# FauxFaux/quadrs

Measured on AMD Instinct MI355X. Metric: Msamples/s through shift->FIR->FFT chain, higher is better.
Workload: dtype f32

## Files before the change

quadrs_amd/build.py:

```python
import os
import subprocess
import sys

HERE = os.path.dirname(os.path.abspath(__file__))
ROOT = os.path.dirname(HERE)
SRC = [(os.path.join(HERE, "csrc", "quadrs_hip.hip"), [])]
DEPS = [s for s, _ in SRC] + [os.path.join(HERE, "csrc", f) for f in ("qd_chain.h", "qd_cascade.h", "qd_device.h", "qd_geometry.h", "qd_registry.h", "qd_summary.h", "qd_pieces.h", "qd_pool.h", "qd_limbs.h", "qd_mean.h", "qd_power.h", "qd_spread.h", "qd_density.h", "qd_bands.h", "qd_paint.h", "qd_lists.h", "qd_bursts.h", "qd_emissions.h", "qd_cuts.h", "qd_cuts_plan.h", "qd_symbols.h", "qd_symbols_plan.h")] + [
    os.path.join(ROOT, "include", "quadrs_hip.h")]
OBJ_DIR = os.path.join(ROOT, "build", "obj")
OUT = os.path.join(HERE, "libquadrs_hip.so")

FLAGS = ["-O3", "--offload-arch=gfx950", "-ffp-contract=off", "-fPIC", "-std=c++17",
         "-fno-fast-math", "-Wall", "-Wno-unused-function", "-I", os.path.join(ROOT, "include"),
         "-Rpass-analysis=kernel-resource-usage",
         "-mllvm", "-amdgpu-atomic-optimizer-strategy=None"]
RESOURCES = os.path.join(ROOT, "build", "kernel_resources.json")


def parse_resource_remarks(text):
    import re
    out, cur = {}, None
    for line in text.splitlines():
        m = re.search(r"remark: Function Name: (\S+)", line)
        if m:
            cur = out.setdefault(m.group(1), {})
            continue
        m = re.search(r"remark:\s+(TotalSGPRs|VGPRs|ScratchSize \[bytes/lane\]|Occupancy \[waves/SIMD\]|SGPRs Spill|VGPRs Spill): (\d+)", line)
        if m and cur is not None:
            cur[m.group(1).split(" [")[0]] = int(m.group(2))
    return out


def hipcc():
    for c in (os.environ.get("HIPCC"), "/opt/rocm/bin/hipcc", "hipcc"):
        if c and (os.path.isabs(c) and os.path.exists(c) or not os.path.isabs(c)):
            return c
    return "hipcc"


def needs_build():
# ... 94 lines not shown
```

quadrs_amd/csrc/qd_cascade.h:

```cpp
#pragma once

#include "qd_chain.h"

namespace qd {

constexpr uint32_t kCascadeRow = 512;
constexpr uint32_t kCascadeThreads = 256;
constexpr uint32_t kCascS0 = 1, kCascS1 = 2, kCascL2 = 4, kCascS2 = 8;

struct CascadeParams {
    ChainParams c;
    const float *h1, *h2;
    const double2 *jtab;
    const RowBase *rows[3];
    uint64_t row0[3];
    double ratio0, ratio1, ratio2;
    uint64_t S;
    uint32_t D1, T1, D2, T2;
    uint32_t n2;
    uint32_t M;
    uint32_t inter_elems, src_elems;
    uint32_t dmagic1, dmagic2;
    uint32_t phi2;
    uint32_t flags;
};

__device__ __forceinline__ uint32_t casc_pad(uint32_t m, uint32_t dmagic, uint32_t phi = 0) { return dmagic ? m + __umulhi(m + phi, dmagic) : m; }

__device__ __forceinline__ int casc_fir_class(uint32_t D) { return (D & 1) ? 0 : (D == 2 ? 2 : (D == 4 ? 4 : (D % 8 == 0 ? 8 : -1))); }

template <int DC>
__device__ __forceinline__ float2 casc_fir_full(const float2 *x, const_f32_p h, uint32_t T, uint32_t D) {
    v2f acc = {0.f, 0.f};
    uint32_t j = 0;
    for (; j + 8 <= T; j += 8) {
        const float2 *xp = x + (DC == 0 ? j : j + j / D);
        float2 xv[8];
        float hv[8];
#pragma unroll
        for (uint32_t u = 0; u < 8; ++u) { xv[u] = xp[(DC == 2 || DC == 4) ? u + u / DC : u]; hv[u] = h[j + u]; }
#pragma unroll
        for (uint32_t u = 0; u < 8; ++u) {
            const v2f xx = {xv[u].x, xv[u].y}, hh = {hv[u], hv[u]};
            acc = acc + xx * hh;
        }
    }
// ... 9 lines not shown
    float ar = 0.f, ai = 0.f;
    for (uint32_t j = 0; j < jmax; ++j) {
        const float2 x = base[casc_pad(q0 + j, dmagic, phi)];
        const float hj = h[j];
        ar = ar + x.x * hj;
        ai = ai + x.y * hj;
    }
    return make_float2(ar, ai);
}

__device__ __forceinline__ float2 casc_fir(int cls, const float2 *base, uint32_t q0, uint32_t jmax, uint32_t T, uint32_t D, const_f32_p h,
                                           uint32_t dmagic, uint32_t phi) {
    if (jmax == T) {
        const float2 *x = base + casc_pad(q0, dmagic, phi);
        switch (cls) {
        case 0: return casc_fir_full<0>(x, h, T, D);
        case 2: return casc_fir_full<2>(x, h, T, D);
        case 4: return casc_fir_full<4>(x, h, T, D);
        case 8: return casc_fir_full<8>(x, h, T, D);
        default: break;
        }
    }
    return casc_fir_any(base, q0, jmax, h, dmagic, phi);
}

template <int FMT>
__device__ __forceinline__ float2 casc_load(const uint8_t *src, uint64_t i) {
    if constexpr (FMT == 0) return reinterpret_cast<const float2 *>(src)[i];
    else if constexpr (FMT == 1) { const uint16_t w = reinterpret_cast<const uint16_t *>(src)[i]; return make_float2(unpack_cs8(w & 0xff), unpack_cs8(w >> 8)); }
    else if constexpr (FMT == 2) { const uint16_t w = reinterpret_cast<const uint16_t *>(src)[i]; return make_float2(unpack_cu8(w & 0xff), unpack_cu8(w >> 8)); }
    else { const uint32_t w = reinterpret_cast<const uint32_t *>(src)[i]; return make_float2(unpack_cs16(w & 0xffffu), unpack_cs16(w >> 16)); }
}

__device__ __forceinline__ float2 casc_nco(const RowBase *rb, uint64_t row0, uint64_t n, const double2 *jt, double ratio) {
    const uint32_t j = (uint32_t)(n % kCascadeRow);
    const double2 cs = jt[j];
    LaneRot lr;
    lr.jf = (double)j; lr.c = cs.x; lr.s = cs.y;
    return nco_mul<true>(rb[n / kCascadeRow - row0], lr, ratio);
}

template <int FMT>
__global__ __launch_bounds__(kCascadeThreads) void k_cascade(const CascadeParams P) {
    extern __shared__ __attribute__((aligned(16))) float2 casc_lds[];
    float2 *inter = casc_lds;
    float2 *tile = casc_lds + P.inter_elems;
    const uint32_t tid = threadIdx.x;
    const ChainParams &C = P.c;
    const DynGeo geo(C);
    const uint32_t D1 = P.D1, T1 = P.T1, D2 = P.D2, T2 = P.T2, n2 = P.n2, W = C.W;
    const uint32_t c1 = T1 - T1 / 2, c2 = T2 - T2 / 2;
    const uint64_t n1 = (uint64_t)n2 * D1 + T1;
    const bool l2 = (P.flags & kCascL2) != 0;
    const_f32_p h1 = (const_f32_p)P.h1;
    const_f32_p h2 = (const_f32_p)P.h2;
    const uint32_t log_width = 2 * geo.layers;
    const int cls1 = casc_fir_class(D1), cls2 = casc_fir_class(D2);
    for (uint64_t w = C.first_window + blockIdx.x; w < C.first_window + C.n_windows; w += gridDim.x) {
        const uint64_t o = w * P.S;
        const uint64_t b2 = l2 ? o * D2 : o;
        const uint64_t b1 = b2 * D1;
        for (uint32_t i0 = 0; i0 < n2; i0 += P.M) {
            const uint32_t m = n2 - i0 < P.M ? n2 - i0 : P.M;
            const uint64_t s0 = b1 + (uint64_t)i0 * D1 + c1;
            const uint64_t want = (uint64_t)(m - 1) * D1 + T1, left = n1 - ((uint64_t)i0 * D1 + c1);
            const uint32_t ns = (uint32_t)(want < left ? want : left);
            __syncthreads();
            for (uint32_t q = tid; q < ns; q += kCascadeThreads) {
                const uint64_t s = s0 + q;
                float2 x = make_float2(0.f, 0.f);
                if (s >= C.src_first && s < C.src_first + C.src_count) x = casc_load<FMT>(C.src, s - C.src_first);
                if (P.flags & kCascS0) x = cmul(x, casc_nco(P.rows[0], P.row0[0], s, P.jtab, P.ratio0));
// ... 120 lines not shown
```

quadrs_amd/csrc/qd_chain.h:

```cpp
#pragma once

#include "qd_device.h"
#include "qd_geometry.h"

namespace qd {

#ifdef QD_STAMP
#define QD_STAMP_DECL unsigned long long st_prev = 0, st_acc[8] = {0, 0, 0, 0, 0, 0, 0, 0}, st_row[4] = {0, 0, 0, 0}; unsigned st_tiles = 0;
#define QD_STAMP_ROW(k) do { unsigned long long t_; asm volatile("s_memtime %0\n\ts_waitcnt lgkmcnt(0)" : "=s"(t_) :: "memory"); st_row[k] += t_ - st_prev; st_acc[0] += t_ - st_prev; st_prev = t_; } while (0)
#define QD_STAMP_START() do { asm volatile("s_memtime %0\n\ts_waitcnt lgkmcnt(0)" : "=s"(st_prev) :: "memory"); } while (0)
#define QD_STAMP_AT(k) do { unsigned long long t_; asm volatile("s_memtime %0\n\ts_waitcnt lgkmcnt(0)" : "=s"(t_) :: "memory"); st_acc[k] += t_ - st_prev; st_prev = t_; } while (0)
#define QD_STAMP_FLUSH() do { if (P.stamps && (threadIdx.x & 63) == 0 && threadIdx.x < 1024) { unsigned w_ = threadIdx.x >> 6; for (int k_ = 0; k_ < 8; ++k_) atomicAdd(&P.stamps[w_ * 8 + k_], st_acc[k_]); if (w_ == 1) for (int k_ = 0; k_ < 4; ++k_) atomicAdd(&P.stamps[129 + k_], st_row[k_]); if (w_ == 0) for (int k_ = 0; k_ < 4; ++k_) atomicAdd(&P.stamps[133 + k_], st_row[k_]); if (w_ == 0) atomicAdd(&P.stamps[128], (unsigned long long)st_tiles); } } while (0)
#define QD_STAMP_TILE() do { ++st_tiles; } while (0)
#else
#define QD_STAMP_DECL
#define QD_STAMP_START()
#define QD_STAMP_AT(k)
#define QD_STAMP_FLUSH()
#define QD_STAMP_TILE()
#define QD_STAMP_ROW(k)
#endif

#ifdef QD_DEVELOP
#define QD_DBG(P, bit) (((P).dbg & (bit)) != 0)
#else
#define QD_DBG(P, bit) false
#endif

typedef const float __attribute__((address_space(4))) *const_f32_p;
typedef const double __attribute__((address_space(4))) *const_f64_p;

template <int FMT> struct FmtTraits;
template <> struct FmtTraits<0> { static constexpr int BPS = 8; static constexpr int SPL = 2; using Vec = uint4; };
template <> struct FmtTraits<1> { static constexpr int BPS = 2; static constexpr int SPL = 4; using Vec = uint2; };
template <> struct FmtTraits<2> { static constexpr int BPS = 2; static constexpr int SPL = 4; using Vec = uint2; };
template <> struct FmtTraits<3> { static constexpr int BPS = 4; static constexpr int SPL = 4; using Vec = uint4; };

struct ChainParams {
    const uint8_t *src;
    uint64_t src_first;
    uint64_t src_count;
    uint64_t first_window;
    uint64_t n_windows;
    uint64_t out_window0;
    void *out;
    const RowBase *rowtab;
    uint64_t rowtab_row0;
    const double2 *jtab;
    const float *taps;
    const float2 *tw;
    double ratio;
    float rmin, rmax;
    float root2;
    float2 tw16_1, tw16_2, tw16_3;
    uint32_t epi;
    float gstep;
    float rgstep;
    uint32_t dbg;
    unsigned long long *stamps;
    unsigned long long *work;
    const uint64_t *row_offsets;
    const float *window;
    uint32_t blk_len;
    uint32_t blk_sub_mask;
    uint32_t tile_extra;
    uint32_t W, logW, S, D, T, G;
    uint32_t Dp;
    uint32_t dmagic;
    uint32_t dshift;
    uint32_t a0, b0;
    uint32_t T_fast;
    uint32_t a1, b1;
    uint32_t base_len, log_base, layers;
    uint32_t lds_raw_elems;
    uint32_t lds_dyn;
    uint32_t out_row_stride;
};

template <class GeoT>
__device__ __forceinline__ uint8_t glyph_of(const ChainParams &P, float nm) {
    if constexpr (GeoT::kFixed) return glyph_code(nm, P.rmin, P.rmax, P.gstep, P.rgstep);
// ... 170 lines not shown
        }
        return *reinterpret_cast<const Vec *>(rowp + t);
    } else {
        const int32_t m0 = g.rel0 + (int32_t)(i * (NT * SPL)) + (int32_t)(tid * SPL);
        uint32_t w[4] = {0, 0, 0, 0};
#pragma unroll
        for (int u = 0; u < SPL; ++u) {
            const int32_t m = m0 + u;
            if (m >= 0 && m < (int32_t)g.tile_raw) {
                const uint8_t *sp = P.src + (g.n_start + (uint32_t)m - P.src_first) * BPS;
                if constexpr (FMT == 0) { uint2 t = *reinterpret_cast<const uint2 *>(sp); w[2 * u] = t.x; w[2 * u + 1] = t.y; }
                else if constexpr (FMT == 3) { w[u] = *reinterpret_cast<const uint32_t *>(sp); }
                else { uint32_t t = *reinterpret_cast<const uint16_t *>(sp); w[u >> 1] |= t << (16 * (u & 1)); }
            }
        }
        Vec v{};
        if constexpr (sizeof(Vec) == 16) { v.x = w[0]; v.y = w[1]; v.z = w[2]; v.w = w[3]; }
        else { v.x = w[0]; v.y = w[1]; }
        return v;
    }
}

template <bool HAS_SHIFT>
__device__ __forceinline__ double prefetch_rowtab(const ChainParams &P, const TileGeo &ng, uint32_t tid) {
    double v = 0.0;
    if constexpr (HAS_SHIFT) {
        uint32_t r = tid < ng.n_rows ? tid : ng.n_rows - 1;
        asm volatile("" : "+v"(r));
        v = P.rowtab[ng.r0 - P.rowtab_row0 + r].c;
    }
    return v;
}

__device__ __forceinline__ RowBase load_rowbase(const ChainParams &P, uint64_t r) {
    const_f64_p rp = (const_f64_p)(uintptr_t)(P.rowtab + (r - P.rowtab_row0));
    RowBase rb;
    rb.c = rp[0]; rb.s = rp[1]; rb.nf = rp[2]; rb.pad_ = 0.0;
    return rb;
}

__device__ __forceinline__ RowBase load_rowbase_at(const_f64_p tile_rows, uint32_t i) {
    RowBase rb;
    rb.c = tile_rows[4 * i + 0]; rb.s = tile_rows[4 * i + 1]; rb.nf = tile_rows[4 * i + 2]; rb.pad_ = 0.0;
    return rb;
}

__device__ __forceinline__ uint32_t opaque_u32(uint32_t v) { asm volatile("" : "+v"(v)); return v; }

template <class GeoT>
__device__ __forceinline__ uint32_t pad_index(const GeoT &geo, uint32_t m) {
    if (geo.Dp == geo.D) return m;
    if (geo.pshift != 0xffffffffu) return m + geo.kPad * (m >> geo.pshift);
    return m + geo.kPad * __umulhi(m, geo.dmagic);
}

template <int FMT, int NT, int NCO, bool INTERIOR, class GeoT>
__device__ __forceinline__ void process_row(const ChainParams &P, const GeoT &geo, const TileGeo &g, int32_t rel,
                                            uint32_t tid, const typename FmtTraits<FMT>::Vec &v, const RowBase &rb,
                                            const LaneRot *lr, uint32_t lane_pad, const float *lut, float2 *raw,
                                            float2 *dup = nullptr, uint32_t dup_limit = 0) {
    using FT = FmtTraits<FMT>;
    constexpr int SPL = FT::SPL;
    constexpr uint32_t ROW = NT * SPL;
    const int32_t m0 = rel + (int32_t)(tid * SPL);
    if constexpr (!INTERIOR) {
        if (!(m0 + SPL > 0 && m0 < (int32_t)g.tile_raw)) return;
    }
    float2 x[SPL];
    if constexpr (FMT == 0) {
        x[0] = make_float2(__uint_as_float(v.x), __uint_as_float(v.y));
        x[1] = make_float2(__uint_as_float(v.z), __uint_as_float(v.w));
    } else if constexpr (FMT == 1) {
        const uint32_t a = v.x ^ 0x80808080u, b = v.y ^ 0x80808080u;
        x[0] = make_float2(unpack_cs8_at(a, 0), unpack_cs8_at(a, 1));
        x[1] = make_float2(unpack_cs8_at(a, 2), unpack_cs8_at(a, 3));
        x[2] = make_float2(unpack_cs8_at(b, 0), unpack_cs8_at(b, 1));
// ... 730 lines not shown

    extern __shared__ __attribute__((aligned(16))) char smem[];
    float2 *raw = reinterpret_cast<float2 *>(smem);
    constexpr bool kDefer = defer_fft_ok<GeoT, HAS_FIR>((uint32_t)NT);
    constexpr bool kQuadFft = quad_fft_ok<GeoT, HAS_FIR>((uint32_t)NT);
    constexpr uint32_t kSlots = GeoT::kBatch;
    constexpr uint32_t kBatch = kDefer ? 1u : GeoT::kBatch;
    constexpr uint32_t kLutElems = (FMT == 1 || FMT == 2) ? 256u : 0u;
    float2 *fb0 = raw + geo.lds_raw_elems;
    float2 *twl = fb0 + (size_t)kSlots * geo.G * geo.W;
    float *tapl = reinterpret_cast<float *>(twl + geo.W);
    float *lut = tapl + ((geo.T + 3) & ~3u);
    float2 *dec = reinterpret_cast<float2 *>(lut + kLutElems);
    float2 *trc = dec + ((geo.G - 1) * geo.S + geo.W);
    uint32_t *bmeta = reinterpret_cast<uint32_t *>(GeoT::kShared ? trc + ((geo.G - 1) * geo.S + geo.W) : dec);
    uint32_t *wq = bmeta + 4 * kSlots;

    const uint32_t tid = threadIdx.x;
    const uint32_t W = geo.W, logW = geo.logW, S = geo.S, D = geo.D, T = geo.T, Dp = geo.Dp;


    constexpr bool kReloadLane = HAS_SHIFT && ((GeoT::kFixed && GeoT::kFirTile > 1) || !GeoT::kFixed);
    constexpr bool kFastP1 = fast_p1_ok<FMT, NT, GeoT>(RCH, WHOLE, ALIGNED);
    constexpr bool kHalf = GeoT::kHalfTile;
    static_assert(!kHalf || (kFastP1 && defer_fft_ok<GeoT, HAS_FIR>((uint32_t)NT)), "half-window tiles: row-aligned phase 1 and the deferred FFT");
    static_assert((GeoT::kFlags & kGeoWindow) == 0 || (GeoT::kFixed && family_of(GeoT::kFlags) == kFamChain), "kGeoWindow: a plan-time build of k_chain");
    static_assert(!GeoT::kWindow || HAS_FIR || GeoT::kFixed, "WinGeo: behind a lowpass only (without one DynGeo tests the pointer)");
    uint32_t half = 0;
    LaneRot lr[SPL];
    auto load_lane_rot = [&](uint32_t first) {
#pragma unroll
        for (int u = 0; u < SPL; ++u) {
            uint32_t j = first + u;
            double2 cs = P.jtab[j];
            lr[u].jf = (double)j;
            lr[u].c = cs.x;
            lr[u].s = cs.y;
        }
    };
    if constexpr (HAS_SHIFT && !kReloadLane) load_lane_rot(tid * SPL);
    const uint32_t lane_pad = pad_index(geo, tid * SPL);
    {
        const uint32_t n_tw = W - geo.base_len;
        for (uint32_t i = tid; i < n_tw; i += NT) twl[i] = P.tw[i];
        if (tid == 0) bmeta[0] = 0;
        for (uint32_t i = tid; i < T; i += NT) tapl[i] = P.taps[i];
    }
    __syncthreads();

    const uint64_t n_tiles = (P.n_windows + geo.G - 1) / geo.G;
    constexpr bool kWinLane = GeoT::kFixed && GeoT::kWindow && GeoT::kPairFir && !kHalf && GeoT::G_ct * GeoT::W_ct <= (uint32_t)NT;
    float win_lane = 1.f;
    if constexpr (kWinLane) win_lane = P.window[tid & (W - 1)];
    auto win_pair = [&](uint32_t k, float2 v) -> float2 {
        if constexpr (kWinLane) { v.x = v.x * win_lane; v.y = v.y * win_lane; return v; }
        else return win_mul<GeoT>(P, k, v);
    };

    uint64_t walk_base = 0, walk_local = blockIdx.x, walk_step = gridDim.x, walk_limit = n_tiles;
    const bool xcd_walk = (gridDim.x & 7u) == 0 && n_tiles >= 8;
    const uint64_t n8 = (n_tiles + 7) / 8;
    auto xcd_limit = [&](uint32_t x) -> uint64_t { const uint64_t b = (uint64_t)x * n8; return b >= n_tiles ? 0 : (n_tiles - b < n8 ? n_tiles - b : n8); };
    if (xcd_walk) {
        walk_base = (uint64_t)(blockIdx.x & 7u) * n8;
        walk_local = blockIdx.x >> 3;
        walk_step = gridDim.x >> 3;
        walk_limit = xcd_limit(blockIdx.x & 7u);
    }
    auto walk_tile = [&](uint64_t local) -> uint64_t { return local < walk_limit ? walk_base + local : n_tiles; };
    const bool dyn = P.work != nullptr && xcd_walk;
// ... 95 lines not shown
            bf4(s0, s1, s2, s3);
            const float n0 = norm_ref(s2), n1 = norm_ref(s3), n2 = norm_ref(s0), n3 = norm_ref(s1);
            if (P.epi == 0) { outf[i] = n0; outf[i + Wq] = n1; outf[i + 2 * Wq] = n2; outf[i + 3 * Wq] = n3; }
            else {
                outb[i] = glyph_of<GeoT>(P, n0); outb[i + Wq] = glyph_of<GeoT>(P, n1);
                outb[i + 2 * Wq] = glyph_of<GeoT>(P, n2); outb[i + 3 * Wq] = glyph_of<GeoT>(P, n3);
            }
        }
    };
    uint32_t bslot = 0;
    QD_STAMP_DECL
    QD_STAMP_START();
    while (tg.valid) {
        const uint64_t w0 = tg.w0;
        const uint32_t g_cnt = tg.g_cnt;

        double rt_pf = 0.0;
        __builtin_amdgcn_s_setprio(0);
        if constexpr (kReloadLane) {
            uint32_t first = tid * SPL;
            asm volatile("" : "+v"(first));
            load_lane_rot(first);
        }
        unsigned long long claim = 0;
        if (dyn && tid == 0 && (!kHalf || half == 1)) claim = atomicAdd(&P.work[16 * my_x], 1ull);
        if constexpr (GeoT::kRows) {
            static_assert(!ALIGNED && !WHOLE, "row mode: the per-sample loads");
            for (uint32_t g = 0; g < g_cnt; ++g) {
                const TileGeo wg = row_window_geo<FMT, NT>(P, geo, tg, g);
                float2 *rawg = raw + (size_t)g * S * Dp;
                for (uint32_t r = 0; r < wg.n_rows; ++r) {
                    const Vec v = fetch_row<FMT, NT, false>(P, wg, r, tid);
                    RowBase rb{};
                    if constexpr (HAS_SHIFT) rb = load_rowbase(P, wg.r0 + r);
                    process_row_any<FMT, NT, NCO>(P, geo, wg, r, tid, v, rb, lr, lane_pad, lut, rawg);
                }
            }
        } else
        if constexpr (kFastP1) {
            constexpr uint32_t ROWB = NT * SPL * FT::BPS, VECB = SPL * FT::BPS;
            constexpr uint32_t kTileRaw = kHalf ? GeoT::kHalfRaw : (GeoT::G - 1) * GeoT::S * GeoT::D + GeoT::W * GeoT::D + GeoT::T;
            constexpr uint32_t kRem = kTileRaw - (RCH - 1) * (NT * SPL);
            constexpr uint32_t kHalfStep = GeoT::kHalfOut * GeoT::D;
            uint64_t tile_pf = tile_n < n_tiles ? tile_n : tile;
            if (kHalf && half == 0) tile_pf = tile;
            const uint64_t ns_n = (P.first_window + tile_pf * GeoT::G) * ((uint64_t)GeoT::S * GeoT::D) + ((kHalf && half == 0) ? kHalfStep : 0u);
            const uint64_t left = (P.src_first + P.src_count - ns_n) * FT::BPS;
            const auto rsrc = __builtin_amdgcn_make_buffer_rsrc(const_cast<uint8_t *>(P.src) + (ns_n - P.src_first) * FT::BPS, 0,
                                                                left > 0xffffffffull ? 0xffffffffu : (uint32_t)left, 0x00020000);
            if constexpr (HAS_SHIFT) {
                uint32_t r = tid < (uint32_t)RCH ? tid : (uint32_t)RCH - 1;
                asm volatile("" : "+v"(r));
                rt_pf = P.rowtab[ns_n / (NT * SPL) - P.rowtab_row0 + r].c;
            }
            const_f64_p rows = (const_f64_p)(uintptr_t)(P.rowtab + (tg.r0 + (kHalf ? half * (kHalfStep / (NT * SPL)) : 0u) - P.rowtab_row0));
            RowBase rb_next{};
            if constexpr (HAS_SHIFT) rb_next = load_rowbase_at(rows, 0);
            TileGeo gl = tg;
            gl.tile_raw = kTileRaw;
#pragma unroll
            for (int i = 0; i < RCH; ++i) {
                const Vec v = pf[i];
                const RowBase rb = rb_next;
                if constexpr (HAS_SHIFT) { if (i + 1 < RCH) rb_next = load_rowbase_at(rows, i + 1); }
                if (i + 1 < RCH || kRem == NT * SPL) {
                    process_row<FMT, NT, NCO, true>(P, geo, gl, i * (NT * SPL), tid, v, rb, lr, lane_pad, lut, raw);
                } else {
                    if (tid * SPL < kRem) process_row<FMT, NT, NCO, (kRem % SPL) == 0>(P, geo, gl, i * (NT * SPL), tid, v, rb, lr, lane_pad, lut, raw);
                }
                __builtin_amdgcn_sched_barrier(0);
                typedef unsigned v4u_t __attribute__((ext_vector_type(4)));
                typedef unsigned v2u_t __attribute__((ext_vector_type(2)));
                constexpr uint32_t kLastVec = ((kRem * FT::BPS - 1) / VECB) * VECB;
                uint32_t voff = tid * VECB;
                if (i + 1 == RCH && kRem != NT * SPL) voff = voff < kLastVec ? voff : kLastVec;
                const bool shared_row = (GeoT::kFlags & kGeoNtInner) && (i == 0 || i + 1 == RCH);
                if constexpr (sizeof(Vec) == 16) {
                    const v4u_t w = shared_row ? __builtin_amdgcn_raw_buffer_load_b128(rsrc, (int)voff, (int)(i * ROWB), 0)
                                               : __builtin_amdgcn_raw_buffer_load_b128(rsrc, (int)voff, (int)(i * ROWB), ct_load_aux(GeoT::kFlags));
                    pf[i].x = w.x; pf[i].y = w.y; pf[i].z = w.z; pf[i].w = w.w;
                } else {
                    const v2u_t w = shared_row ? __builtin_amdgcn_raw_buffer_load_b64(rsrc, (int)voff, (int)(i * ROWB), 0)
                                               : __builtin_amdgcn_raw_buffer_load_b64(rsrc, (int)voff, (int)(i * ROWB), ct_load_aux(GeoT::kFlags));
                    pf[i].x = w.x; pf[i].y = w.y;
                }
                __builtin_amdgcn_sched_barrier(0);
            }
        } else
        if constexpr (WHOLE) {
            TileGeo ng = tile_geo<FMT, NT>(P, geo, tile_n, n_tiles);
            if (!ng.valid) ng = tg;
            rt_pf = prefetch_rowtab<HAS_SHIFT>(P, ng, tid);
            RowBase rb_next{};
            if constexpr (HAS_SHIFT) rb_next = load_rowbase(P, tg.r0);
#pragma unroll
            for (int i = 0; i < RCH; ++i) {
                const Vec v = pf[i];
#ifdef QD_STAMP
                asm volatile("" :: "v"(v.x), "v"(v.y));
                QD_STAMP_ROW(0);
#endif
                if ((uint32_t)i < tg.n_rows) {
                    const RowBase rb = rb_next;
#ifdef QD_STAMP
                    asm volatile("" :: "s"(rb.c), "s"(rb.nf));
                    QD_STAMP_ROW(2);
#endif
                    if constexpr (HAS_SHIFT) {
                        if ((uint32_t)i + 1 < tg.n_rows) rb_next = load_rowbase(P, tg.r0 + i + 1);
                    }
                    process_row_any<FMT, NT, NCO>(P, geo, tg, i, tid, v, rb, lr, lane_pad, lut, raw);
                    QD_STAMP_ROW(3);
                }
                __builtin_amdgcn_sched_barrier(0);
                pf[i] = fetch_row<FMT, NT, ALIGNED, (GeoT::kFlags & kGeoNtLoads) != 0>(P, ng, (uint32_t)i < ng.n_rows ? i : ng.n_rows - 1, tid);
                QD_STAMP_ROW(1);
                __builtin_amdgcn_sched_barrier(0);
            }
        } else {
            for (uint32_t r = 0; r < tg.n_rows; r += RCH) {
                Vec cur[RCH];
#pragma unroll
                for (int i = 0; i < RCH; ++i) cur[i] = pf[i];
                TileGeo ng = tg;
                uint32_t rbase = r + RCH;
                if (rbase >= tg.n_rows) {
                    const TileGeo t2 = tile_geo<FMT, NT>(P, geo, tile_n, n_tiles);
                    if (t2.valid) { ng = t2; rbase = 0; rt_pf = prefetch_rowtab<HAS_SHIFT>(P, t2, tid); } else { rbase = tg.n_rows - 1; }
                }
#pragma unroll
                for (int i = 0; i < RCH; ++i)
                    pf[i] = fetch_row<FMT, NT, ALIGNED, (GeoT::kFlags & kGeoNtLoads) != 0>(P, ng, rbase + i < ng.n_rows ? rbase + i : ng.n_rows - 1, tid);
                RowBase rb[RCH];
#pragma unroll
                for (int i = 0; i < RCH; ++i) {
                    rb[i] = RowBase{};
                    if constexpr (HAS_SHIFT) { if (r + i < tg.n_rows) rb[i] = load_rowbase(P, tg.r0 + r + i); }
                }
#pragma unroll
                for (int i = 0; i < RCH; ++i)
                    if (r + i < tg.n_rows) process_row_any<FMT, NT, NCO>(P, geo, tg, r + i, tid, cur[i], rb[i], lr, lane_pad, lut, raw);
            }
        }
        QD_STAMP_AT(0);
        __syncthreads();
        QD_STAMP_AT(1);

        __builtin_amdgcn_s_setprio(1);
        if constexpr (kDefer) {
            constexpr uint32_t GW = GeoT::G_ct * GeoT::W_ct, GWP = kHalf ? GeoT::kHalfOut : GW, FL = GeoT::kPackedTile ? GWP / 2 : GWP;
            float2 *fb_cur = fb0 + (size_t)dpar * GW, *fb_prev = fb0 + (size_t)(dpar ^ 1u) * GW;
            const uint32_t n_out_d = kHalf ? GWP : (g_cnt << logW);
            const uint32_t log_width_d = 2 * geo.layers;
            const uint32_t k_first = kHalf ? half * GWP : 0u;
            if (tid < FL) {
                if constexpr (GeoT::kPackedTile) {
                    const uint32_t o0 = tid * 2;
                    if (o0 < n_out_d) {
                        const uint32_t g = kHalf ? 0u : (o0 >> logW), k0 = kHalf ? k_first + o0 : (o0 & (W - 1));
                        uint32_t jm[2];
#pragma unroll
                        for (int r = 0; r < 2; ++r) { const uint32_t j2 = (W - (k0 + r)) * D + T / 2; jm[r] = j2 < T ? j2 : T; }
                        float2 full[2], snp[2];
                        const uint32_t q0 = kHalf ? o0 : g * S + k0;
                        if ((tid >> 8) & 1u) fir_tiled2_pk<GeoT, 1>(raw + (q0 * D + GeoT::kPad * (q0 / 2)), tapl, full, jm, snp); else fir_tiled2_pk<GeoT, 0>(raw + (q0 * D + GeoT::kPad * (q0 / 2)), tapl, full, jm, snp);
#pragma unroll
                        for (int r = 0; r < 2; ++r) {
                            const uint32_t k = k0 + r;
                            const uint32_t xx = k & ((1u << log_width_d) - 1), yy = k >> log_width_d;
                            fb_cur[(g << logW) + yy + (rev4(xx, geo.layers) << geo.log_base)] = win_mul<GeoT>(P, k, jm[r] < T ? snp[r] : full[r]);
                        }
                    }
                } else if (tid < n_out_d) {
                    const uint32_t g = kHalf ? 0u : (tid >> logW), k = kHalf ? k_first + tid : (tid & (W - 1));
// ... 462 lines not shown
    auto claim_resolve = [&](unsigned long long got) -> uint64_t {
        uint32_t mx = my_x;
        asm volatile("" : "+s"(mx));
        const uint64_t dyn_base = 3 * walk_step;
        if (got + dyn_base < xcd_limit(mx)) return (uint64_t)mx * n8 + dyn_base + got;
#pragma unroll 1
        for (uint32_t k = 1; k < 8; ++k) {
            const uint32_t xx = (mx + k) & 7u;
            const uint64_t lim = xcd_limit(xx);
            if (lim <= dyn_base) continue;
            const unsigned long long i = atomicAdd(&P.work[16 * xx], 1ull);
            if (i + dyn_base < lim) return (uint64_t)xx * n8 + dyn_base + i;
        }
        return n_tiles;
    };
    uint64_t tile_x = n_tiles, tile_f = walk_tile(walk_local), tile_p = walk_tile(walk_local + walk_step), tile_pn = walk_tile(walk_local + 2 * walk_step);
    walk_local += 2 * walk_step;
    auto next_after = [&]() -> uint64_t {
        if (dyn) return ((uint64_t)__builtin_amdgcn_readfirstlane(wq[1]) << 32) | __builtin_amdgcn_readfirstlane(wq[0]);
        walk_local += walk_step;
        return walk_tile(walk_local);
    };
    auto g_cnt_of = [&](uint64_t t) -> uint32_t {
        const uint64_t w0 = t * G, left = P.n_windows - w0;
        return left < G ? (uint32_t)left : G;
    };

    if (wave < 8) {
        LaneRot lr[SPL];
        if constexpr (HAS_SHIFT) {
#pragma unroll
            for (int u = 0; u < SPL; ++u) {
                const uint32_t j = tid * SPL + u;
                const double2 cs = P.jtab[j];
                lr[u].jf = (double)j; lr[u].c = cs.x; lr[u].s = cs.y;
            }
        }
        const uint32_t lane_pad = pad_index(geo, tid * SPL);
        typedef unsigned v4u_t __attribute__((ext_vector_type(4)));
        typedef unsigned v2u_t __attribute__((ext_vector_type(2)));
        auto n_start_of = [&](uint64_t t) -> uint64_t { return (P.first_window + t * G) * ((uint64_t)S * D); };
        auto rsrc_of = [&](uint64_t t) {
            const uint64_t ns = n_start_of(t);
            const uint64_t left = (P.src_first + P.src_count - ns) * FT::BPS;
            return __builtin_amdgcn_make_buffer_rsrc(const_cast<uint8_t *>(P.src) + (ns - P.src_first) * FT::BPS, 0,
                                                     left > 0xffffffffull ? 0xffffffffu : (uint32_t)left, 0x00020000);
        };
        Vec pf[RCH];
        auto load_row = [&](const decltype(rsrc_of(0)) &rsrc, int i) {
            constexpr uint32_t kLastVec = ((kRem * FT::BPS - 1) / VECB) * VECB;
            uint32_t voff = tid * VECB;
            if (i + 1 == RCH && kRem != ROW) voff = voff < kLastVec ? voff : kLastVec;
            constexpr int aux = ct_load_aux(GeoT::kFlags);
            const bool shared_row = (GeoT::kFlags & kGeoNtInner) && (i == 0 || i + 1 == RCH);
            if constexpr (sizeof(Vec) == 16) {
                const v4u_t w = shared_row ? __builtin_amdgcn_raw_buffer_load_b128(rsrc, (int)voff, (int)(i * ROWB), 0)
                                           : __builtin_amdgcn_raw_buffer_load_b128(rsrc, (int)voff, (int)(i * ROWB), aux);
                pf[i].x = w.x; pf[i].y = w.y; pf[i].z = w.z; pf[i].w = w.w;
            } else {
                const v2u_t w = shared_row ? __builtin_amdgcn_raw_buffer_load_b64(rsrc, (int)voff, (int)(i * ROWB), 0)
                                           : __builtin_amdgcn_raw_buffer_load_b64(rsrc, (int)voff, (int)(i * ROWB), aux);
                pf[i].x = w.x; pf[i].y = w.y;
            }
        };
        double rt_touch = 0.0;
        auto produce = [&](uint64_t t_cur, uint64_t t_refill, float2 *rawbuf) {
            const uint64_t ns = n_start_of(t_cur);
            const uint64_t t_pf = t_refill < n_tiles ? t_refill : t_cur;
// ... 253 lines not shown
    float2 *fbx = raw + K::FBX_OFF;
    float2 *twl = fbx + 2 * (size_t)G * W;
    float *tapl = reinterpret_cast<float *>(kWrite ? raw + K::RAW_ELEMS : twl + W);
    if (P.lds_dyn < K::kLdsBytes) return;

    const uint32_t tid = threadIdx.x;
    const uint32_t wave = __builtin_amdgcn_readfirstlane(tid >> 6);
    {
        if constexpr (!kWrite) {
            const uint32_t n_tw = W - geo.base_len;
            for (uint32_t i = tid; i < n_tw; i += NTHR) twl[i] = P.tw[i];
        }
        for (uint32_t i = tid; i < T; i += NTHR) tapl[i] = P.taps[i];
    }
    __syncthreads();

    const uint64_t n_tiles = (P.n_windows + G - 1) / G;
    const uint64_t base_cnt = n_tiles / gridDim.x, rem = n_tiles % gridDim.x;
    const uint64_t t_lo = (uint64_t)blockIdx.x * base_cnt + (blockIdx.x < rem ? blockIdx.x : rem);
    const uint32_t n_steps = (uint32_t)(base_cnt + (blockIdx.x < rem ? 1u : 0u));
    if (n_steps == 0) return;
    const uint32_t n_iter = n_steps + (kWrite ? 2u : 4u);
    auto g_cnt_of = [&](uint64_t t) -> uint32_t {
        const uint64_t w0 = t * G, left = P.n_windows - w0;
        return left < G ? (uint32_t)left : G;
    };

    if (wave < PW) {
        LaneRot lr[SPL];
        if constexpr (HAS_SHIFT) {
#pragma unroll
            for (int u = 0; u < SPL; ++u) {
                const uint32_t j = tid * SPL + u;
                const double2 cs = P.jtab[j];
                lr[u].jf = (double)j; lr[u].c = cs.x; lr[u].s = cs.y;
            }
        }
        const uint32_t lane_pad = pad_index(geo, tid * SPL);
        typedef unsigned v4u_t __attribute__((ext_vector_type(4)));
        typedef unsigned v2u_t __attribute__((ext_vector_type(2)));
        const uint64_t n0 = (P.first_window + t_lo * G) * ((uint64_t)S * D);
        auto rsrc_of = [&](uint32_t step1) {
            const uint64_t ns = n0 + (uint64_t)step1 * K::N;
            const uint64_t end = P.src_first + P.src_count;
            const uint64_t left = ns < end ? (end - ns) * FT::BPS : 0;
            return __builtin_amdgcn_make_buffer_rsrc(const_cast<uint8_t *>(P.src) + (ns - P.src_first) * FT::BPS, 0,
                                                     left > 0xffffffffull ? 0xffffffffu : (uint32_t)left, 0x00020000);
        };
        Vec pf[RN];
        auto load_row = [&](const decltype(rsrc_of(0)) &rsrc, int i) {
            constexpr int aux = ct_load_aux(GeoT::kFlags);
            if constexpr (sizeof(Vec) == 16) {
                const v4u_t w = __builtin_amdgcn_raw_buffer_load_b128(rsrc, (int)(tid * VECB), (int)(i * ROWB), aux);
                pf[i].x = w.x; pf[i].y = w.y; pf[i].z = w.z; pf[i].w = w.w;
            } else {
                const v2u_t w = __builtin_amdgcn_raw_buffer_load_b64(rsrc, (int)(tid * VECB), (int)(i * ROWB), aux);
                pf[i].x = w.x; pf[i].y = w.y;
            }
        };
        double rt_touch = 0.0;
        TileGeo gl{};
        gl.tile_raw = ROW;
        __builtin_amdgcn_s_setprio(0);
        {
            const auto rsrc = rsrc_of(0);
#pragma unroll
            for (int i = 0; i < (int)RN; ++i) load_row(rsrc, i);
        }
// ... 177 lines not shown
                                const float nm = norm_ref(spark_ld2(fb + ((e ^ SZ::delta(e)) << 3)));
                                if (P.epi == 0) outf[o] = nm;
                                else outb[o] = glyph_of<GeoT>(P, nm);
                            }
                        }
                    } else
                    wave_fft_epilogue_fn<GeoT, (GH * W + 63) / 64, 2>(P, geo, twl, fbp, P.first_window + t * G + g0, g1 - g0, tid);
                }
            }
            __syncthreads();
        }
    }
}


struct SparkWalk {
    uint64_t first, stride, end;
    __device__ __forceinline__ SparkWalk(uint64_t n_tiles, uint32_t wave) {
        constexpr uint32_t WPG = kThreads / 64;
        if ((gridDim.x & 7u) == 0 && n_tiles >= 64) {
            const uint64_t n8 = (n_tiles + 7) / 8, lo = (uint64_t)(blockIdx.x & 7u) * n8;
            first = lo + (uint64_t)(blockIdx.x >> 3) * WPG + wave;
            stride = (uint64_t)(gridDim.x >> 3) * WPG;
            end = lo + n8 < n_tiles ? lo + n8 : n_tiles;
            if (lo >= n_tiles) { first = n_tiles; end = n_tiles; }
        } else {
            first = (uint64_t)blockIdx.x * WPG + wave; stride = (uint64_t)gridDim.x * WPG; end = n_tiles;
        }
    }
};

template <class GeoT, bool F = GeoT::kFixed> struct W_CT_GE8 { static constexpr bool value = false; };
template <class GeoT> struct W_CT_GE8<GeoT, true> { static constexpr bool value = GeoT::W >= 8; };
template <int FMT> struct SparkTraits {
    using FT = FmtTraits<FMT>;
    static constexpr uint32_t SPL = FT::SPL, CH = 64u * SPL, RQ = kSparkRow / CH;
};

template <int FMT, int NCO, class GeoT, int NCH, int LB, int EPI = -1 >
__global__ __launch_bounds__(kThreads, LB) void k_spark(const ChainParams P) {
    static_assert((GeoT::kFlags & kGeoWindow) == 0, "kGeoWindow: only k_chain applies the plan's window; this kernel would ignore it");
    using FT = FmtTraits<FMT>;
    using Vec = typename FT::Vec;
    using ST = SparkTraits<FMT>;
    constexpr int SPL = FT::SPL;
    constexpr bool HAS_SHIFT = NCO != 0;
    constexpr uint32_t CH = ST::CH, RQ = ST::RQ, TS = (uint32_t)NCH * CH, CHB = CH * FT::BPS, VECB = SPL * FT::BPS;
    static_assert(TS % kSparkRow == 0 && (NCH % RQ) == 0, "a tile is a whole number of NCO rows");
    const GeoT geo(P);
    const uint32_t W = geo.W, logW = geo.logW;
    const uint32_t G = TS >> logW;

    extern __shared__ __attribute__((aligned(16))) char smem[];
    float2 *twl = reinterpret_cast<float2 *>(smem);
    const uint32_t tid = threadIdx.x, lane = tid & 63u;
    const uint32_t wave = __builtin_amdgcn_readfirstlane(tid >> 6);
    constexpr bool kLdsLane = HAS_SHIFT && GeoT::kFixed;
    double2 *jt = reinterpret_cast<double2 *>(twl + (W < 32u ? 32u : W));
    float2 *fbw = twl + (W < 32u ? 32u : W) + (kLdsLane ? 2u * kSparkRow : 0u) + (size_t)wave * TS;
    {
        const uint32_t n_tw = W - geo.base_len;
        for (uint32_t i = tid; i < n_tw; i += kThreads) twl[i] = P.tw[i];
        if constexpr (kLdsLane) { for (uint32_t i = tid; i < kSparkRow; i += kThreads) jt[i] = P.jtab[i]; }
    }
    __syncthreads();

    uint32_t pos[NCH * SPL];
    {
        const uint32_t log_width = 2 * geo.layers;
#pragma unroll
        for (int c = 0; c < NCH; ++c)
#pragma unroll
            for (int u = 0; u < SPL; ++u) {
                const uint32_t m = (uint32_t)c * CH + lane * SPL + (uint32_t)u, k = m & (W - 1);
                const uint32_t xx = k & ((1u << log_width) - 1), yy = k >> log_width;
                pos[c * SPL + u] = (m & ~(W - 1)) + yy + (rev4(xx, geo.layers) << geo.log_base);
            }
    }
    constexpr bool kLeanEpi = GeoT::kFixed && (EPI == 0 || EPI == 1 || EPI == 2);
    const uint32_t fb_off = (uint32_t)(uintptr_t)(__attribute__((address_space(3))) void *)fbw;
    if (kLeanEpi && (fb_off & 255u)) __builtin_trap();
    if constexpr (kLeanEpi) {
        if constexpr (GeoT::W >= 8) {
            using SZ = SparkSwzFn<SparkSwz<GeoT::W, (uint32_t)SPL>>;
#pragma unroll
            for (int i = 0; i < NCH * SPL; ++i) pos[i] ^= SZ::delta(pos[i]);
        }
    }
    double2 lcs[HAS_SHIFT && !kLdsLane ? RQ * SPL : 1];
    double ljf[HAS_SHIFT ? SPL : 1];
    if constexpr (HAS_SHIFT) {
        if constexpr (!kLdsLane) {
#pragma unroll
            for (uint32_t q = 0; q < RQ; ++q)
#pragma unroll
                for (int u = 0; u < SPL; ++u) lcs[q * SPL + u] = P.jtab[q * CH + lane * SPL + (uint32_t)u];
        }
#pragma unroll
        for (int u = 0; u < SPL; ++u) ljf[u] = (double)(lane * SPL + (uint32_t)u);
    }

    const uint64_t n_tiles = (P.n_windows + G - 1) / G;
    SparkWalk walk(n_tiles, wave);
    uint64_t tile = walk.first;
    const uint64_t n_waves = walk.stride, tile_end = walk.end;
    if (tile >= tile_end) return;
    typedef unsigned v4u_t __attribute__((ext_vector_type(4)));
    typedef unsigned v2u_t __attribute__((ext_vector_type(2)));
    auto rsrc_of = [&](uint64_t t) {
        const uint64_t ns = (P.first_window + t * G) << logW, end = P.src_first + P.src_count;
        const uint64_t left = ns < end ? (end - ns) * FT::BPS : 0;
        return __builtin_amdgcn_make_buffer_rsrc(const_cast<uint8_t *>(P.src) + (ns - P.src_first) * FT::BPS, 0,
                                                 left > 0xffffffffull ? 0xffffffffu : (uint32_t)left, 0x00020000);
    };
    Vec pf[NCH];
    auto load_chunk = [&](const decltype(rsrc_of(0)) &rsrc, int c) {
        constexpr int aux = 2;
        if constexpr (sizeof(Vec) == 16) {
            const v4u_t w = __builtin_amdgcn_raw_buffer_load_b128(rsrc, (int)(lane * VECB), (int)(c * CHB), aux);
            pf[c].x = w.x; pf[c].y = w.y; pf[c].z = w.z; pf[c].w = w.w;
        } else {
            const v2u_t w = __builtin_amdgcn_raw_buffer_load_b64(rsrc, (int)(lane * VECB), (int)(c * CHB), aux);
// ... 26 lines not shown
        if constexpr (HAS_SHIFT) rows = (const_f64_p)(uintptr_t)(P.rowtab + (((w0 << logW) / kSparkRow) - P.rowtab_row0));
        RowBase rb{};
#pragma unroll
        for (int c = 0; c < NCH; ++c) {
            const Vec v = pf[c];
            if constexpr (HAS_SHIFT) { if (c % (int)RQ == 0) rb = load_rowbase_at(rows, c / (int)RQ); }
            float2 x[SPL];
            if constexpr (FMT == 0) {
                x[0] = make_float2(__uint_as_float(v.x), __uint_as_float(v.y));
                x[1] = make_float2(__uint_as_float(v.z), __uint_as_float(v.w));
            } else if constexpr (FMT == 1) {
                const uint32_t a = v.x ^ 0x80808080u, b = v.y ^ 0x80808080u;
                x[0] = make_float2(unpack_cs8_at(a, 0), unpack_cs8_at(a, 1));
                x[1] = make_float2(unpack_cs8_at(a, 2), unpack_cs8_at(a, 3));
                x[2] = make_float2(unpack_cs8_at(b, 0), unpack_cs8_at(b, 1));
                x[3] = make_float2(unpack_cs8_at(b, 2), unpack_cs8_at(b, 3));
            } else if constexpr (FMT == 2) {
                x[0] = make_float2(unpack_cu8_at(v.x, 0), unpack_cu8_at(v.x, 1));
                x[1] = make_float2(unpack_cu8_at(v.x, 2), unpack_cu8_at(v.x, 3));
                x[2] = make_float2(unpack_cu8_at(v.y, 0), unpack_cu8_at(v.y, 1));
                x[3] = make_float2(unpack_cu8_at(v.y, 2), unpack_cu8_at(v.y, 3));
            } else {
                x[0] = make_float2(unpack_cs16(v.x & 0xffffu), unpack_cs16(v.x >> 16));
                x[1] = make_float2(unpack_cs16(v.y & 0xffffu), unpack_cs16(v.y >> 16));
                x[2] = make_float2(unpack_cs16(v.z & 0xffffu), unpack_cs16(v.z >> 16));
                x[3] = make_float2(unpack_cs16(v.w & 0xffffu), unpack_cs16(v.w >> 16));
            }
            if constexpr (HAS_SHIFT) {
                float2 m[SPL];
                const int q = c % (int)RQ;
                LaneRot lr[SPL];
#pragma unroll
                for (int u = 0; u < SPL; ++u) {
                    const double2 cs = kLdsLane ? jt[(uint32_t)q * CH + lane * SPL + (uint32_t)u] : lcs[kLdsLane ? 0 : q * SPL + u];
                    lr[u].jf = ljf[u]; lr[u].c = cs.x; lr[u].s = cs.y;
                }
                RowBase rbq = rb;
                rbq.nf = rb.nf + (double)(q * (int)CH);
                nco_mul_n<NCO == 2, SPL>(rbq, lr, P.ratio, m);
#pragma unroll
                for (int u = 0; u < SPL; ++u) x[u] = cmul_pk(x[u], m[u]);
            }
#pragma unroll
            for (int u = 0; u < SPL; ++u) fbw[pos[c * SPL + u]] = x[u];
            __builtin_amdgcn_sched_barrier(0);
            load_chunk(rsrc_n, c);
            __builtin_amdgcn_sched_barrier(0);
        }
        wsync();
        if constexpr (kLean) {
            if constexpr (GeoT::W >= 8) spark_fft_swz<GeoT, TS, (uint32_t)SPL>(P, twl, fb_off, lane);
            else wave_fft_epilogue_fn<GeoT, 0, 3>(P, geo, twl, fbw, w0, G, tid);
            if constexpr (EPI == 2) {
                using SZB = SparkSwzFn<SparkSwz<GeoT::W, (uint32_t)SPL>>;
                uint32_t lo = lane;
                asm volatile("" : "+v"(lo));
                const uint32_t b0 = fb_off + ((lo ^ SZB::delta(lo)) << 3);
                float nmv[NB];
#pragma unroll
                for (uint32_t k = 0; k < NB; ++k) {
                    const uint32_t ec = 64 * k;
                    nmv[k] = norm_ref(spark_ld2((b0 ^ (SZB::delta(ec) << 3)) + (ec << 3)));
                }
                wsync();
                float *nb = reinterpret_cast<float *>(fbw);
#pragma unroll
                for (uint32_t k = 0; k < NB; ++k) nb[lo + 64 * k] = nmv[k];
                wsync();
// ... 58 lines not shown



template <uint32_t W> struct Spark2Swz { static constexpr uint32_t m[4] = {0, 0, 0, 0}; };
template <> struct Spark2Swz<128> { static constexpr uint32_t m[4] = {0x40, 0x10, 0x20, 0x40}; };
template <> struct Spark2Swz<256> { static constexpr uint32_t m[4] = {0x80, 0x10, 0x20, 0x40}; };
template <> struct Spark2Swz<512> { static constexpr uint32_t m[4] = {0x100, 0x20, 0x60, 0x40}; };
template <> struct Spark2Swz<1024> { static constexpr uint32_t m[4] = {0x200, 0x40, 0x80, 0x40}; };
template <int FMT> struct Spark2Raw { using type = uint32_t; };
template <> struct Spark2Raw<0> { typedef unsigned type __attribute__((ext_vector_type(4))); };
template <> struct Spark2Raw<3> { typedef unsigned type __attribute__((ext_vector_type(2))); };
template <class GeoT> struct Spark2 {
    static constexpr uint32_t W = GeoT::W, base = GeoT::base_len, layers = GeoT::layers, width = W / base;
    static constexpr uint32_t LPW = width / 2, GW = 64 / (LPW ? LPW : 1), TS = GW * W, NBF = TS / 256;
    static constexpr bool ok = GeoT::kFixed && GeoT::R.spark2_ok();
    static constexpr uint32_t kRows = TS / kSparkRow;
};

template <int FMT, int NCO, class GeoT, int LB, int EPI >
__global__ __launch_bounds__(kThreads, LB) void k_spark2(const ChainParams P) {
    static_assert((GeoT::kFlags & kGeoWindow) == 0, "kGeoWindow: only k_chain applies the plan's window; this kernel would ignore it");
    using K = Spark2<GeoT>;
    using FT = FmtTraits<FMT>;
    static_assert(K::ok, "k_spark2: W = base * 16 or base * 64");
    constexpr bool HAS_SHIFT = NCO != 0;
    constexpr uint32_t S = GeoT::S;
    static_assert(S == K::W || !HAS_SHIFT, "k_spark2: overlapping windows only without a shift (the NCO rows are laid out for whole tiles)");
    constexpr uint32_t BPS = FT::BPS;
    constexpr uint32_t W = K::W, logW = GeoT::logW, base = K::base, layers = K::layers, width = K::width, LPW = K::LPW, GW = K::GW, TS = K::TS, NBF = K::NBF;
    const GeoT geo(P);

    extern __shared__ __attribute__((aligned(16))) char smem[];
    float2 *twl = reinterpret_cast<float2 *>(smem);
    double2 *jt = reinterpret_cast<double2 *>(twl + W);
    const uint32_t tid = threadIdx.x, lane = tid & 63u;
    const uint32_t wave = __builtin_amdgcn_readfirstlane(tid >> 6);
    float2 *fbw = twl + W + (HAS_SHIFT ? 2u * kSparkRow : 0u) + (size_t)wave * TS;
    for (uint32_t i = tid; i < W - base; i += kThreads) twl[i] = P.tw[i];
    if constexpr (HAS_SHIFT) { for (uint32_t i = tid; i < kSparkRow; i += kThreads) jt[i] = P.jtab[i]; }
    __syncthreads();

    constexpr bool kSwz = EPI != 2;
    using SZ = SparkSwzFn<Spark2Swz<kSwz ? W : 0u>>;
    const uint32_t fb = (uint32_t)(uintptr_t)(__attribute__((address_space(3))) void *)fbw;
    if (fb & 255u) __builtin_trap();
    const uint32_t g = lane / LPW, xp = lane % LPW;
    const uint32_t r0 = g * W + (rev4(2 * xp, layers) << GeoT::log_base), r1 = g * W + (rev4(2 * xp + 1, layers) << GeoT::log_base);
    const uint32_t p0 = fb + ((r0 ^ SZ::delta(r0)) << 3), p1 = fb + ((r1 ^ SZ::delta(r1)) << 3);
    const uint64_t n_tiles = (P.n_windows + GW - 1) / GW;
    SparkWalk walk(n_tiles, wave);
    uint64_t tile = walk.first;
    const uint64_t n_waves = walk.stride, tile_end = walk.end;
    if (tile >= tile_end) return;
    typedef unsigned v4u_t __attribute__((ext_vector_type(4)));
    typedef unsigned v2u_t __attribute__((ext_vector_type(2)));
    auto rsrc_of = [&](uint64_t t) {
        const uint64_t ns = (P.first_window + t * GW) * S, end = P.src_first + P.src_count;
        const uint64_t left = ns < end ? (end - ns) * BPS : 0;
        return __builtin_amdgcn_make_buffer_rsrc(const_cast<uint8_t *>(P.src) + (ns - P.src_first) * BPS, 0,
                                                 left > 0xffffffffull ? 0xffffffffu : (uint32_t)left, 0x00020000);
    };
    const uint32_t voff = (g * S + 2 * xp) * BPS;
    using Raw = typename Spark2Raw<FMT>::type;
    Raw raw[base];
    auto load_rows = [&](const decltype(rsrc_of(0)) &rsrc) {
#pragma unroll
        for (uint32_t y = 0; y < base; ++y) {
            if constexpr (FMT == 0) raw[y] = __builtin_amdgcn_raw_buffer_load_b128(rsrc, (int)voff, (int)(y * width * BPS), 2 );
            else if constexpr (FMT == 3) raw[y] = __builtin_amdgcn_raw_buffer_load_b64(rsrc, (int)voff, (int)(y * width * BPS), 2);
            else raw[y] = __builtin_amdgcn_raw_buffer_load_b32(rsrc, (int)voff, (int)(y * width * BPS), 2);
// ... 18 lines not shown
    while (true) {
        const uint64_t tile_n = tile + n_waves;
        const uint64_t w0 = P.first_window + tile * GW, left_w = P.first_window + P.n_windows - w0;
        const uint32_t g_cnt = left_w < GW ? (uint32_t)left_w : GW;
        constexpr uint32_t OBW = EPI == 0 ? 4u * W : (EPI == 4 ? 1u : W);
        const uint32_t RS = P.out_row_stride ? P.out_row_stride : 1u;
        const auto orsrc = __builtin_amdgcn_make_buffer_rsrc(reinterpret_cast<uint8_t *>(P.out) + (w0 - P.out_window0) * RS * OBW, 0,
                                                             g_cnt ? ((g_cnt - 1) * RS + 1) * OBW : 0u, 0x00020000);
        RowBase rbl[W > kSparkRow ? W / kSparkRow : 1];
        if constexpr (HAS_SHIFT) {
            const_f64_p rows = (const_f64_p)(uintptr_t)(P.rowtab + (((w0 << logW) / kSparkRow) - P.rowtab_row0));
            constexpr uint32_t RPW = W > kSparkRow ? W / kSparkRow : 1;
#pragma unroll
            for (uint32_t h = 0; h < RPW; ++h) {
                const uint32_t ridx = W >= kSparkRow ? g * RPW + h : (g * W) / kSparkRow;
                RowBase sel = load_rowbase_at(rows, 0);
#pragma unroll
                for (uint32_t r = 1; r < K::kRows; ++r) {
                    const RowBase cand = load_rowbase_at(rows, r);
                    if (ridx == r) sel = cand;
                }
                rbl[h] = sel;
            }
        }
#pragma unroll
        for (int u = 0; u < 2; ++u) {
            float2 v[base];
#pragma unroll
            for (uint32_t y = 0; y < base; ++y) {
                float2 x = column(y, u);
                if constexpr (HAS_SHIFT) {
                    const uint32_t jrow = (W >= kSparkRow ? 0u : (g * W) % kSparkRow) + (y * width) % kSparkRow;
                    const uint32_t j = jrow + 2 * xp + (uint32_t)u;
                    const double2 cs = jt[j];
                    LaneRot lr; lr.jf = (double)j; lr.c = cs.x; lr.s = cs.y;
                    const RowBase &rb = rbl[W > kSparkRow ? (y * width) / kSparkRow : 0];
                    x = cmul_pk(x, nco_mul<NCO == 2>(rb, lr, P.ratio));
                }
                v[y] = x;
            }
#if !(defined(QD_SPARK_ABL) && (QD_SPARK_ABL & 8))
            if constexpr (base == 16) bf16(v, P.tw16_1, P.tw16_2, P.tw16_3, P.root2); else bf8(v, P.root2);
#endif
            const uint32_t pb = u == 0 ? p0 : p1;
#pragma unroll
            for (uint32_t q = 0; q < base / 2; ++q)
                *(spark_lds_f4 *)(uintptr_t)(pb ^ (16 * q)) = spark_f4n{v[2 * q].x, v[2 * q].y, v[2 * q + 1].x, v[2 * q + 1].y};
            __builtin_amdgcn_sched_barrier(0);
        }
        __builtin_amdgcn_sched_barrier(0);
        load_rows(rsrc_of(tile_n < tile_end ? tile_n : tile));
        __builtin_amdgcn_sched_barrier(0);
        uint32_t cols = base, log_cols = GeoT::log_base, tw_off = 0;
        uint32_t marks = 0;
        uint32_t lo = lane;
        asm volatile("" : "+v"(lo));
#pragma unroll
        for (uint32_t l = 0; l < layers; ++l) {
            wsync();
#if defined(QD_SPARK_ABL) && (QD_SPARK_ABL & 4)
            if (l + 1 < layers) { tw_off += 3 * cols; cols *= 4; log_cols += 2; continue; }
#endif
            const bool last = l + 1 == layers;
            float2 tc1 = make_float2(0.f, 0.f), tc2 = tc1, tc3 = tc1;
            if (cols <= 64) { const uint32_t i = lo & (cols - 1); tc1 = twl[tw_off + 3 * i]; tc2 = twl[tw_off + 3 * i + 1]; tc3 = twl[tw_off + 3 * i + 2]; }
            constexpr uint32_t KB = 2;
#pragma unroll
            for (uint32_t k0 = 0; k0 < NBF; k0 += KB) {
// ... 204 lines not shown
```

quadrs_amd/csrc/qd_cuts.h:

```cpp
#pragma once

#include "qd_cuts_plan.h"

#if defined(__HIPCC__)
#include "qd_device.h"

namespace qd {

constexpr uint32_t kCutShift = 1, kCutSecondOrder = 2;

struct __attribute__((aligned(16))) CutJob {
    double ratio;
    uint64_t span0, valid;
    uint64_t taps_at, lane_at;
    uint32_t D, T, flags, _pad;
};

__device__ __forceinline__ void cut_tile_reads(const CutJob &jb, const CutTile &tl, uint64_t *lo, uint64_t *hi) {
    const uint64_t ctr = jb.T - jb.T / 2;
    *lo = (uint64_t)tl.first * jb.D + ctr;
    const uint64_t end = (uint64_t)(tl.first + tl.count - 1) * jb.D + ctr + jb.T;
    *hi = end < jb.valid ? end : jb.valid;
}

__global__ __launch_bounds__(256) void k_cuts_tables(const CutJob *__restrict__ jobs, const CutTile *__restrict__ tiles, uint32_t n_tiles, RowBase *__restrict__ rowtab,
                                                    const double *__restrict__ lane_ratio, uint32_t n_lane, double2 *__restrict__ lanetab) {
    const uint64_t i = (uint64_t)blockIdx.x * blockDim.x + threadIdx.x;
    const uint64_t n_row = (uint64_t)n_tiles * kCutsTileRows;
    if (i < n_row) {
        const uint32_t t = (uint32_t)(i / kCutsTileRows), r = (uint32_t)(i % kCutsTileRows);
        const CutTile tl = tiles[t];
        const CutJob jb = jobs[tl.job];
        if (!(jb.flags & kCutShift)) return;
        uint64_t lo, hi;
        cut_tile_reads(jb, tl, &lo, &hi);
        const uint64_t row = (jb.span0 + lo) / kCutsNcoRow + r;
        if (row * kCutsNcoRow >= jb.span0 + hi) return;
        RowBase rb;
        rb.nf = (double)(row * kCutsNcoRow);
        rb.pad_ = 0.0;
        nco_table_entry(rb.nf, jb.ratio, &rb.c, &rb.s);
        rowtab[i] = rb;
    } else if (i - n_row < (uint64_t)n_lane * kCutsNcoRow) {
        const uint64_t u = (i - n_row) / kCutsNcoRow, j = (i - n_row) % kCutsNcoRow;
        double c, s;
        nco_table_entry((double)j, lane_ratio[u], &c, &s);
        lanetab[u * kCutsNcoRow + j] = make_double2(c, s);
    }
}

template <int FMT> constexpr int cuts_bps() { return FMT == QD_FMT_CF32 ? 8 : (FMT == QD_FMT_CS16 ? 4 : 2); }

template <int FMT>
__device__ __forceinline__ float2 cuts_load(const uint8_t *p) {
    if constexpr (FMT == QD_FMT_CF32) {
        return *reinterpret_cast<const float2 *>(p);
    } else if constexpr (FMT == QD_FMT_CS16) {
        const uint32_t w = *reinterpret_cast<const uint32_t *>(p);
        return make_float2(unpack_cs16(w & 0xffffu), unpack_cs16(w >> 16));
    } else {
        const uint32_t w = *reinterpret_cast<const uint16_t *>(p);
        return FMT == QD_FMT_CS8 ? make_float2(unpack_cs8(w & 0xffu), unpack_cs8(w >> 8)) : make_float2(unpack_cu8(w & 0xffu), unpack_cu8(w >> 8));
    }
}

template <int FMT>
__device__ __forceinline__ void cuts_load_vec(const uint8_t *p, float2 *s) {
    const uint4 q = *reinterpret_cast<const uint4 *>(p);
    const uint32_t w[4] = {q.x, q.y, q.z, q.w};
    if constexpr (FMT == QD_FMT_CF32) {
        s[0] = make_float2(__builtin_bit_cast(float, w[0]), __builtin_bit_cast(float, w[1]));
        s[1] = make_float2(__builtin_bit_cast(float, w[2]), __builtin_bit_cast(float, w[3]));
    } else if constexpr (FMT == QD_FMT_CS16) {
#pragma unroll
        for (int u = 0; u < 4; ++u) s[u] = make_float2(unpack_cs16(w[u] & 0xffffu), unpack_cs16(w[u] >> 16));
    } else {
#pragma unroll
        for (int u = 0; u < 8; ++u) {
            const uint32_t h = (w[u >> 1] >> (16 * (u & 1))) & 0xffffu;
            s[u] = FMT == QD_FMT_CS8 ? make_float2(unpack_cs8(h & 0xffu), unpack_cs8(h >> 8)) : make_float2(unpack_cu8(h & 0xffu), unpack_cu8(h >> 8));
        }
    }
}

template <int FMT>
__global__ __launch_bounds__(kCutsThreads) void k_cuts(const uint8_t *__restrict__ src, const CutJob *__restrict__ jobs, const CutTile *__restrict__ tiles,
                                                       const float *__restrict__ taps, const RowBase *__restrict__ rowtab,
                                                       const double2 *__restrict__ lanetab, float2 *__restrict__ out) {
    extern __shared__ __attribute__((aligned(32))) char smem_cuts[];
    RowBase *rows = reinterpret_cast<RowBase *>(smem_cuts);
    float2 *xs = reinterpret_cast<float2 *>(smem_cuts + kCutsTileRows * sizeof(RowBase));
    constexpr int BPS = cuts_bps<FMT>(), SPV = 16 / BPS;
    const uint32_t tid = threadIdx.x;
    const CutTile tl = tiles[blockIdx.x];
    const CutJob jb = jobs[tl.job];
    uint64_t rel0, rel1;
    cut_tile_reads(jb, tl, &rel0, &rel1);
    uint32_t len = (uint32_t)(rel1 - rel0);
    if (len > kCutsTileSamples) len = kCutsTileSamples;
    const uint64_t abs0 = jb.span0 + rel0, row0 = abs0 / kCutsNcoRow;
    const bool shift = (jb.flags & kCutShift) != 0, second = (jb.flags & kCutSecondOrder) != 0;
    if (shift && tid < kCutsTileRows) rows[tid] = rowtab[(uint64_t)blockIdx.x * kCutsTileRows + tid];
    __syncthreads();

    auto put = [&](uint32_t k, float2 v) {
        if (shift) {
            const uint64_t n = abs0 + k;
            const uint32_t j = (uint32_t)(n % kCutsNcoRow);
            const RowBase rb = rows[(uint32_t)(n / kCutsNcoRow - row0)];
            const double2 cs = lanetab[jb.lane_at + j];
            LaneRot lr;
            lr.jf = (double)j; lr.c = cs.x; lr.s = cs.y;
            const float2 m = second ? nco_mul<true>(rb, lr, jb.ratio) : nco_mul<false>(rb, lr, jb.ratio);
            v = cmul(v, m);
        }
        xs[cuts_lds_index(k)] = v;
    };
    const uint8_t *p0 = src + ((int64_t)abs0 + tl.src_off) * BPS;
    uint32_t head = (uint32_t)(((16u - (uint32_t)((uintptr_t)p0 & 15u)) & 15u) / BPS);
    if (head > len || ((uintptr_t)p0 & (BPS - 1))) head = len;
    const uint32_t n_vec = (len - head) / SPV, tail = head + n_vec * SPV;
    for (uint32_t k = tid; k < head; k += kCutsThreads) put(k, cuts_load<FMT>(p0 + (size_t)k * BPS));
    for (uint32_t v = tid; v < n_vec; v += kCutsThreads) {
        float2 s[SPV];
        cuts_load_vec<FMT>(p0 + ((size_t)head + (size_t)v * SPV) * BPS, s);
#pragma unroll
        for (int u = 0; u < SPV; ++u) put(head + v * SPV + u, s[u]);
    }
    for (uint32_t k = tail + tid; k < len; k += kCutsThreads) put(k, cuts_load<FMT>(p0 + (size_t)k * BPS));
    __syncthreads();

    if (tid < tl.count) {
        const uint32_t T = jb.T;
        const uint64_t base = (uint64_t)(tl.first + tid) * jb.D + (T - T / 2);
        const uint64_t left = jb.valid - base;
        const uint32_t jmax = left < T ? (uint32_t)left : T;
        const uint32_t k0 = tid * jb.D;
        const float *__restrict__ h = taps + jb.taps_at;
        float ar = 0.f, ai = 0.f;
        for (uint32_t j = 0; j < jmax; ++j) {
            const float2 x = xs[cuts_lds_index(k0 + j)];
            const float hj = h[j];
            ar = ar + x.x * hj;
            ai = ai + x.y * hj;
        }
// ... 7 lines not shown
```

quadrs_amd/csrc/qd_device.h:

```cpp
#pragma once

#if !defined(__HIPCC_RTC__)
#include <hip/hip_runtime.h>
#include <stdint.h>
#else
typedef unsigned char uint8_t; typedef signed char int8_t; typedef unsigned short uint16_t; typedef short int16_t;
typedef unsigned int uint32_t; typedef int int32_t; typedef unsigned long long uint64_t; typedef long long int64_t;
typedef unsigned long uintptr_t; typedef unsigned long size_t;
#endif

namespace qd {


__device__ __forceinline__ float2 cmul(float2 a, float2 b) {
    float2 r;
    r.x = a.x * b.x - a.y * b.y;
    r.y = a.x * b.y + a.y * b.x;
    return r;
}
__device__ __forceinline__ float2 cmul_pk(float2 a, float2 b) {
    typedef float v2f_t __attribute__((ext_vector_type(2)));
    const v2f_t av = {a.x, a.y}, bv = {b.x, b.y};
    v2f_t r, t;
    asm("v_pk_mul_f32 %0, %2, %3 op_sel_hi:[0,1]\n\t"
// ... 104 lines not shown
    bf4(b0, b1, b2, b3);
    b1 = cscale(cadd(rot90(b1), b1), root2);
    b2 = rot90(b2);
    b3 = cscale(csub(rot90(b3), b3), root2);
    bf2(a0, b0); bf2(a1, b1); bf2(a2, b2); bf2(a3, b3);
    v[0] = a0; v[1] = a1; v[2] = a2; v[3] = a3;
    v[4] = b0; v[5] = b1; v[6] = b2; v[7] = b3;
}

__device__ __forceinline__ void bf16(float2 *v, float2 tw1, float2 tw2, float2 tw3, float root2) {
    float2 ev[8] = { v[0], v[2], v[4], v[6], v[8], v[10], v[12], v[14] };
    float2 p0 = v[1], p1 = v[5], p2 = v[9], p3 = v[13];
    float2 q0 = v[15], q1 = v[3], q2 = v[7], q3 = v[11];
    bf8(ev, root2);
    bf4(p0, p1, p2, p3);
    bf4(q0, q1, q2, q3);
    p1 = cmul(p1, tw1); q1 = cmul(q1, cconj(tw1));
    p2 = cmul(p2, tw2); q2 = cmul(q2, cconj(tw2));
    p3 = cmul(p3, tw3); q3 = cmul(q3, cconj(tw3));
    bf2(p0, q0); bf2(p1, q1); bf2(p2, q2); bf2(p3, q3);
    q0 = rot90(q0); q1 = rot90(q1); q2 = rot90(q2); q3 = rot90(q3);
    v[0] = cadd(ev[0], p0); v[1] = cadd(ev[1], p1); v[2] = cadd(ev[2], p2); v[3] = cadd(ev[3], p3);
    v[4] = cadd(ev[4], q0); v[5] = cadd(ev[5], q1); v[6] = cadd(ev[6], q2); v[7] = cadd(ev[7], q3);
    v[8] = csub(ev[0], p0); v[9] = csub(ev[1], p1); v[10] = csub(ev[2], p2); v[11] = csub(ev[3], p3);
    v[12] = csub(ev[4], q0); v[13] = csub(ev[5], q1); v[14] = csub(ev[6], q2); v[15] = csub(ev[7], q3);
}

__device__ __forceinline__ uint32_t rev4(uint32_t x, uint32_t digits) {
    uint32_t r = 0;
    for (uint32_t d = 0; d < digits; ++d) { r = (r << 2) | (x & 3u); x >>= 2; }
    return r;
}


struct __attribute__((aligned(32))) RowBase {
    double c, s;
    double nf;
    double pad_;
};

struct LaneRot { double jf, c, s; };

__device__ __forceinline__ void nco_table_entry(double kf, double ratio, double *c, double *s) {
    const double th = kf * ratio;
    const double lo = __builtin_fma(kf, ratio, -th);
    double s0, c0;
    sincos(th, &s0, &c0);
    const double q = 0.5 * lo * lo, sl = __builtin_fma(-lo * lo * lo, 1.0 / 6.0, lo);
    *c = c0 + __builtin_fma(-q, c0, -sl * s0);
    *s = s0 + __builtin_fma(-q, s0, sl * c0);
}

template <bool SECOND_ORDER>
__device__ __forceinline__ float2 nco_mul(const RowBase &rb, const LaneRot &lr, double ratio) {
    const double nf = rb.nf + lr.jf;
    const double place = nf * ratio;
    const double r = __builtin_fma(nf, ratio, -place);
    const double C = __builtin_fma(-rb.s, lr.s, rb.c * lr.c);
    const double S = __builtin_fma(rb.s, lr.c, rb.c * lr.s);
    double c, s;
    if constexpr (SECOND_ORDER) {
        const double h = 0.5 * r;
        c = __builtin_fma(r, __builtin_fma(-h, C, S), C);
        s = __builtin_fma(-r, __builtin_fma(h, S, C), S);
    } else {
        c = __builtin_fma(r, S, C);
        s = __builtin_fma(-r, C, S);
    }
    return make_float2((float)c, (float)s);
}

template <bool SECOND_ORDER, int N>
__device__ __forceinline__ void nco_mul_n(const RowBase &rb, const LaneRot *lr, double ratio, float2 *m) {
    double nf[N], pl[N], r[N], C[N], S[N], c[N], s[N];
#pragma unroll
    for (int u = 0; u < N; ++u) nf[u] = rb.nf + lr[u].jf;
#pragma unroll
    for (int u = 0; u < N; ++u) { pl[u] = nf[u] * ratio; C[u] = rb.c * lr[u].c; S[u] = rb.c * lr[u].s; }
#pragma unroll
    for (int u = 0; u < N; ++u) { r[u] = __builtin_fma(nf[u], ratio, -pl[u]); C[u] = __builtin_fma(-rb.s, lr[u].s, C[u]); S[u] = __builtin_fma(rb.s, lr[u].c, S[u]); }
    if constexpr (SECOND_ORDER) {
        double h[N], uu[N], vv[N];
#pragma unroll
        for (int u = 0; u < N; ++u) h[u] = 0.5 * r[u];
#pragma unroll
        for (int u = 0; u < N; ++u) { uu[u] = __builtin_fma(-h[u], C[u], S[u]); vv[u] = __builtin_fma(h[u], S[u], C[u]); }
#pragma unroll
        for (int u = 0; u < N; ++u) { c[u] = __builtin_fma(r[u], uu[u], C[u]); s[u] = __builtin_fma(-r[u], vv[u], S[u]); }
    } else {
#pragma unroll
        for (int u = 0; u < N; ++u) { c[u] = __builtin_fma(r[u], S[u], C[u]); s[u] = __builtin_fma(-r[u], C[u], S[u]); }
    }
#pragma unroll
    for (int u = 0; u < N; ++u) m[u] = make_float2((float)c[u], (float)s[u]);
}

}
```

quadrs_amd/csrc/qd_geometry.h:

```cpp
#pragma once

#if !defined(__HIPCC_RTC__)
#include <stdint.h>
#else
typedef unsigned char uint8_t; typedef signed char int8_t; typedef unsigned short uint16_t; typedef short int16_t;
typedef unsigned int uint32_t; typedef int int32_t; typedef unsigned long long uint64_t; typedef long long int64_t;
#endif

namespace qd {

constexpr uint32_t kGeoNoSplit = 4;
constexpr uint32_t kGeoFastP1 = 8;
constexpr uint32_t kGeoUnrolledFir = 32;
constexpr uint32_t kGeoDeferFft = 64;
constexpr uint32_t kGeoPackedTile = 128;
constexpr uint32_t kGeoNtLoads = 256;
constexpr uint32_t kGeoHalfTile = 8192;
constexpr uint32_t kGeoFastFma = 16384;
constexpr uint32_t kGeoPipe3 = 32768;
constexpr uint32_t kGeoNtInner = 65536;
constexpr uint32_t kGeoStream = 131072;
constexpr uint32_t kGeoWriteSink = 262144;
constexpr uint32_t kGeoSpark = 524288;
constexpr uint32_t kGeoSparkReg = 1048576;
constexpr uint32_t kGeoSparkDirect = 2097152;
constexpr uint32_t kGeoWindow = 1u << 22;

constexpr uint32_t kHintGeoBits = kGeoNoSplit | kGeoFastP1 | kGeoUnrolledFir | kGeoDeferFft | kGeoPackedTile | kGeoNtLoads | kGeoHalfTile | kGeoFastFma |
                                  kGeoPipe3 | kGeoNtInner | kGeoStream | kGeoWriteSink;

constexpr int ct_load_aux(uint32_t flags) { return (flags & kGeoNtLoads) ? 2 : 0; }

constexpr int kThreads = 256;
constexpr int kPipe3Threads = 1024, kPipe3Prod = 512;
constexpr uint32_t kSparkRow = 512;
constexpr uint32_t kSparkMaxW = 1024;

enum Family { kFamChain, kFamPipe3, kFamPipe3s, kFamSpark, kFamSpark2, kFamSpark0 };

constexpr Family family_of(uint32_t flags) {
    return (flags & kGeoSpark) ? ((flags & kGeoSparkDirect) ? kFamSpark0 : (flags & kGeoSparkReg) ? kFamSpark2 : kFamSpark)
         : (flags & kGeoPipe3) ? ((flags & kGeoStream) ? kFamPipe3s : kFamPipe3) : kFamChain;
}

struct FamilyRow {
    const char *name;
    bool on_rows;
};
constexpr FamilyRow kFamilies[] = {
    {"qd::k_chain", false}, {"qd::k_chain_pipe3", true}, {"qd::k_chain_pipe3s", true},
    {"qd::k_spark", true},  {"qd::k_spark2", true},      {"qd::k_spark0", true},
};
constexpr const char *family_name(uint32_t flags) { return kFamilies[family_of(flags)].name; }
constexpr bool row_aligned(uint32_t flags) { return kFamilies[family_of(flags)].on_rows || (flags & kGeoFastP1) != 0; }
constexpr int family_threads(int nt, uint32_t flags) {
    switch (family_of(flags)) {
    case kFamPipe3: return nt + 512;
    case kFamPipe3s: return nt + ((flags & kGeoWriteSink) ? 256 : 512);
    case kFamChain: return nt;
    default: return kThreads;
    }
}

constexpr uint32_t ct_log2(uint64_t v) { uint32_t l = 0; while ((1ull << l) < v) ++l; return l; }
constexpr bool ct_pow2(uint64_t v) { return v && !(v & (v - 1)); }
constexpr uint64_t ct_min(uint64_t a, uint64_t b) { return a < b ? a : b; }
constexpr uint64_t ct_max(uint64_t a, uint64_t b) { return a > b ? a : b; }
constexpr uint64_t ct_gcd(uint64_t a, uint64_t b) { while (b) { const uint64_t t = a % b; a = b; b = t; } return a; }
constexpr uint64_t ct_rows(uint64_t samples, uint64_t row) { return (samples + row - 1) / row; }
// ... 111 lines not shown
    k.RINGD = k.RR * (k.ROW / D);
    k.MIRD = (g.b0 + T + D - 1) / D + 1;
    k.ROWP = (k.ROW / D) * g.Dp;
    k.RAW_ELEMS = ((k.RINGD + k.MIRD) * g.Dp + 1) & ~1ull;
    k.DR = 3 * k.GS;
    k.kOverlap = S < W;
    k.fir_ok = k.kOverlap ? (g.kShared && g.kUnrolledShared)
                          : (S == W && g.kPad == 2 && T % 4 == 0 && g.b0 % 2 == 0 && D % 4 == 0 && T / 4 > 3 && (T / 2) % 4 == 0);
    k.ok = k.fir_ok && k.GS <= 256 && k.GS >= 1 && k.N % k.ROW == 0 && k.ROW % D == 0 && D % spl == 0 && W <= 64 * 16 && k.f0 >= 1 && k.f0 <= k.GS &&
           k.f0 > W - S && g.kNtrunc <= S && k.MIRD * D <= k.ROW && g.Q <= 2 * k.GS;
    k.kWrite = (g.flags & kGeoWriteSink) != 0;
    const uint64_t rings = k.RAW_ELEMS + (k.kOverlap ? 2u : 1u) * k.DR;
    k.FBX_OFF = (rings + 31u) & ~31ull;
    k.FBX_ALIGN = k.FBX_OFF - rings;
    k.kLdsBytes = k.kWrite ? k.RAW_ELEMS * 8 + ct_taps_bytes(T) : (k.FBX_OFF + 2 * G * W + W) * 8 + ct_taps_bytes(T);
    k.GH = (G + 1) / 2;
    k.kSwzFft = !k.kWrite && W >= 8 && (k.GH * W) % 32 == 0 && (G * W) % 32 == 0;
    k.kConsumerThreads = k.kWrite ? 256u : 512u;
    return k;
}

constexpr uint64_t chain_lds_bytes(const FixedRules &g, bool lut8) {
    return g.lds_raw_alloc * 8 + g.kBatch * g.G * g.W * 8 + g.W * 8 + ct_taps_bytes(g.T) + (lut8 ? 256 * 4 : 0) +
           ((g.T && g.S < g.W) ? 2 * g.Q * 8 : 0) + g.kBatch * 16 + 16;
}
constexpr uint64_t generic_raw_elems(const FixedRules &g) { return ct_tile_elems(g.tile_raw, g.D, g.G * g.W, 1); }
constexpr uint64_t generic_lds_bytes(const FixedRules &g, bool lut8) {
    return generic_raw_elems(g) * 8 + g.G * g.W * 8 + g.W * 8 + ct_taps_bytes(g.T) + (lut8 ? 256 * 4 : 0) + ((g.T && g.S < g.W) ? 2 * g.Q * 8 : 0) + 16 + 16;
}
constexpr uint64_t kPipe3QueueBytes = 8;
constexpr uint64_t pipe3_lds_bytes(const FixedRules &g) {
    return 2 * g.lds_raw_alloc * 8 + 4 * g.pipe3_q_pad() * 8 + g.G * g.W * 8 + g.W * 8 + ct_taps_bytes(g.T) + kPipe3QueueBytes;
}
constexpr uint64_t spark_lds_bytes(uint64_t W, uint64_t ts, bool lane_table) { return (ct_max(W, 32) + 4 * ts) * 8 + (lane_table ? kSparkRow * 16 : 0); }
constexpr uint64_t kPipe3LdsSlack = 64 - kPipe3QueueBytes, kStreamLdsSlack = 320, kStreamWriteLdsSlack = 64;
static_assert(31 * 8 < kStreamLdsSlack, "the streaming layout's slack covers FBX_OFF's rounding");

}
```

quadrs_amd/csrc/quadrs_hip.hip:

```cpp
#include <hip/hip_runtime.h>
#include <hip/hiprtc.h>

#include <dlfcn.h>
#include <map>
#include <cmath>
#include <cstdarg>
#include <cstdio>
#include <cstring>
#include <cstdlib>
#include <functional>
#include <memory>
#include <mutex>
#include <numeric>
#include <optional>
#include <thread>
#include <algorithm>
#include <sys/stat.h>
#include <time.h>
#include <unistd.h>
#include <tuple>
#include <string>
#include <vector>

#include "../../include/quadrs_hip.h"
// ... 24 lines not shown
    va_list ap;
    va_start(ap, fmt);
    vsnprintf(buf, sizeof buf, fmt, ap);
    va_end(ap);
    g_err = buf;
    return code;
}

#define HIPCHK(expr)                                                                          \
    do {                                                                                      \
        hipError_t e__ = (expr);                                                              \
        if (e__ != hipSuccess) return fail(QD_ERR_HIP, "%s -> %s", #expr, hipGetErrorString(e__)); \
    } while (0)

constexpr double kPi64 = 3.14159265358979323846264338327950288;
constexpr float kPi32 = 3.14159265358979323846264338327950288f;

#ifdef QD_DEVELOP
const char *dev_env(const char *name) { return getenv(name); }
#else
const char *dev_env(const char *) { return nullptr; }
#endif

uint32_t ilog2(uint64_t v) { uint32_t l = 0; while ((1ull << l) < v) ++l; return l; }
bool is_pow2(uint64_t v) { return v && !(v & (v - 1)); }

int spl_of(int fmt) { return fmt == QD_FMT_CF32 ? 2 : 4; }
int bps_of(int fmt) { return fmt == QD_FMT_CF32 ? 8 : (fmt == QD_FMT_CS16 ? 4 : 2); }


__global__ void k_rowtab(double ratio, uint32_t row_len, uint64_t row0, uint64_t n_rows, uint64_t n_off, RowBase *out) {
    uint64_t i = (uint64_t)blockIdx.x * blockDim.x + threadIdx.x;
    if (i >= n_rows) return;
    RowBase rb;
    rb.nf = (double)((row0 + i) * (uint64_t)row_len + n_off);
    rb.pad_ = 0.0;
    nco_table_entry(rb.nf, ratio, &rb.c, &rb.s);
    out[i] = rb;
}

__global__ void k_jtab(double ratio, uint32_t n, double2 *out) {
    uint32_t j = blockIdx.x * blockDim.x + threadIdx.x;
    if (j >= n) return;
    double s, c;
    nco_table_entry((double)j, ratio, &c, &s);
    out[j] = make_double2(c, s);
}

__global__ void k_unpack(int fmt, const uint8_t *src, size_t n, float2 *out) {
    for (size_t i = (size_t)blockIdx.x * blockDim.x + threadIdx.x; i < n; i += (size_t)gridDim.x * blockDim.x) {
        float2 v;
        switch (fmt) {
        case 0: v = *reinterpret_cast<const float2 *>(src + i * 8); break;
        case 1: { uint16_t w = *reinterpret_cast<const uint16_t *>(src + i * 2); v = make_float2(unpack_cs8(w & 0xff), unpack_cs8(w >> 8)); break; }
        case 2: { uint16_t w = *reinterpret_cast<const uint16_t *>(src + i * 2); v = make_float2(unpack_cu8(w & 0xff), unpack_cu8(w >> 8)); break; }
        default: { uint32_t w = *reinterpret_cast<const uint32_t *>(src + i * 4); v = make_float2(unpack_cs16(w & 0xffffu), unpack_cs16(w >> 16)); break; }
        }
        out[i] = v;
    }
}

__global__ __launch_bounds__(256) void k_shift(float2 *buf, uint64_t abs_off, uint64_t n, double ratio,
                                                const RowBase *rowtab, uint64_t row0, uint64_t n_rows,
                                                const double2 *jtab, int second_order) {
    constexpr uint32_t ROW = 512;
    const uint32_t tid = threadIdx.x;
    LaneRot lr[2];
    for (int u = 0; u < 2; ++u) {
        uint32_t j = tid * 2 + u;
        double2 cs = jtab[j];
        lr[u].jf = (double)j; lr[u].c = cs.x; lr[u].s = cs.y;
    }
    for (uint64_t r = blockIdx.x; r < n_rows; r += gridDim.x) {
        const RowBase rb = rowtab[r];
        for (int u = 0; u < 2; ++u) {
            uint64_t idx = (row0 + r) * ROW + tid * 2 + u;
            if (idx >= abs_off && idx < abs_off + n) {
                float2 m = second_order ? nco_mul<true>(rb, lr[u], ratio) : nco_mul<false>(rb, lr[u], ratio);
                buf[idx - abs_off] = cmul(buf[idx - abs_off], m);
            }
        }
    }
}

__global__ void k_lowpass_block(const float *__restrict__ taps, uint32_t T, uint64_t D, const float2 *__restrict__ raw,
                                uint64_t valid, float2 *out, uint64_t out_n) {
    const uint64_t c = T - T / 2;
    for (uint64_t k = (uint64_t)blockIdx.x * blockDim.x + threadIdx.x; k < out_n; k += (uint64_t)gridDim.x * blockDim.x) {
        uint64_t base = k * D + c;
        uint64_t jmax = valid - base < T ? valid - base : T;
        float ar = 0.f, ai = 0.f;
        for (uint64_t j = 0; j < jmax; ++j) {
            float2 x = raw[base + j];
            float h = taps[j];
            ar = ar + x.x * h;
            ai = ai + x.y * h;
        }
        out[k] = make_float2(ar, ai);
    }
}

__global__ void k_gen(const int64_t *cos_hz, uint32_t n_cos, uint64_t sample_rate, uint64_t first, size_t n, float2 *out) {
    const double tau = kPi64 * 2.0;
    for (size_t i = (size_t)blockIdx.x * blockDim.x + threadIdx.x; i < n; i += (size_t)gridDim.x * blockDim.x) {
        double base = (double)(first + i) * tau / (double)sample_rate;
        float vr = 0.f, vi = 0.f;
        for (uint32_t k = 0; k < n_cos; ++k) {
            double f = (double)cos_hz[k] * base;
            double s, c;
            sincos(f, &s, &c);
            vr = vr + (float)c;
            vi = vi + (float)s;
        }
        out[i] = make_float2(vr, vi);
    }
}

__device__ __forceinline__ double2 zmul(double2 a, double2 b) {
    return make_double2(__builtin_fma(a.x, b.x, -(a.y * b.y)), __builtin_fma(a.x, b.y, a.y * b.x));
}
struct BlueSrc {
    const uint8_t *in; uint64_t in_first;
    double ratio; const RowBase *rowtab; uint64_t rowtab_row0; const double2 *jtab;
};
template <int FMT, int NCO>
__global__ __launch_bounds__(256) void k_bluestein(const BlueSrc src, const uint64_t *__restrict__ offs,
                                                   const float *__restrict__ win, uint32_t W, uint32_t M, uint32_t logM,
                                                   const double2 *__restrict__ chirp, const double2 *__restrict__ Bbr,
                                                   const double2 *__restrict__ tw, float *__restrict__ out) {
    extern __shared__ __attribute__((aligned(16))) char smem_b[];
    double2 *buf = reinterpret_cast<double2 *>(smem_b);
    const uint32_t tid = threadIdx.x;
    const uint64_t row = blockIdx.x;
    const uint64_t n0 = offs[row];
    for (uint32_t n = tid; n < M; n += 256) {
        double2 v = make_double2(0.0, 0.0);
        if (n < W) {
            const uint64_t na = n0 + n;
            const uint8_t *sp = src.in + (na - src.in_first) * (uint64_t)FmtTraits<FMT>::BPS;
            float2 xv;
            if constexpr (FMT == 0) xv = *reinterpret_cast<const float2 *>(sp);
            else if constexpr (FMT == 1) { const uint32_t w = *reinterpret_cast<const uint16_t *>(sp); xv = make_float2(unpack_cs8(w & 0xff), unpack_cs8(w >> 8)); }
            else if constexpr (FMT == 2) { const uint32_t w = *reinterpret_cast<const uint16_t *>(sp); xv = make_float2(unpack_cu8(w & 0xff), unpack_cu8(w >> 8)); }
            else { const uint32_t w = *reinterpret_cast<const uint32_t *>(sp); xv = make_float2(unpack_cs16(w & 0xffffu), unpack_cs16(w >> 16)); }
            if constexpr (NCO != 0) {
                const uint32_t j = (uint32_t)(na & 511u);
                const RowBase rb = src.rowtab[(na >> 9) - src.rowtab_row0];
                const double2 cs = src.jtab[j];
                LaneRot lr; lr.jf = (double)j; lr.c = cs.x; lr.s = cs.y;
                xv = cmul_pk(xv, nco_mul<NCO == 2>(rb, lr, src.ratio));
            }
            if (win) xv = cscale(xv, win[n]);
            v = zmul(make_double2((double)xv.x, (double)xv.y), chirp[n]);
        }
        buf[n] = v;
    }
    __syncthreads();
    for (uint32_t sh = logM; sh-- > 0;) {
        const uint32_t h = 1u << sh;
        for (uint32_t t = tid; t < M / 2; t += 256) {
            const uint32_t j = t & (h - 1), i = ((t >> sh) << (sh + 1)) | j;
            const double2 u = buf[i], v = buf[i + h];
            buf[i] = make_double2(u.x + v.x, u.y + v.y);
            buf[i + h] = zmul(make_double2(u.x - v.x, u.y - v.y), tw[j << (logM - 1 - sh)]);
        }
        __syncthreads();
    }
    for (uint32_t r = tid; r < M; r += 256) buf[r] = zmul(buf[r], Bbr[r]);
    __syncthreads();
    for (uint32_t sh = 0; sh < logM; ++sh) {
        const uint32_t h = 1u << sh;
        for (uint32_t t = tid; t < M / 2; t += 256) {
            const uint32_t j = t & (h - 1), i = ((t >> sh) << (sh + 1)) | j;
            const double2 w = tw[j << (logM - 1 - sh)];
            const double2 u = buf[i], v = zmul(buf[i + h], make_double2(w.x, -w.y));
            buf[i] = make_double2(u.x + v.x, u.y + v.y);
            buf[i + h] = make_double2(u.x - v.x, u.y - v.y);
        }
        __syncthreads();
    }
    const uint32_t half = W / 2;
    for (uint32_t k = tid; k < W; k += 256) {
// ... 25 lines not shown
float2 compute_twiddle(size_t index, size_t fft_len) {
    double constant = -2.0 * kPi64 / (double)fft_len;
    double angle = constant * (double)index;
    return make_float2((float)std::cos(angle), (float)std::sin(angle));
}

struct FftLayout {
    uint32_t base_len = 1, log_base = 0, layers = 0;
    std::vector<float2> tw;
};

FftLayout fft_layout(uint64_t W) {
    FftLayout L;
    uint32_t e = ilog2(W);
    uint32_t be = e <= 3 ? e : ((e & 1) ? 3 : 4);
    L.log_base = be; L.base_len = 1u << be; L.layers = (e - be) / 2;
    size_t cross = L.base_len;
    while (cross < W) {
        size_t cols = cross;
        cross *= 4;
        for (size_t i = 0; i < cols; ++i)
            for (size_t k = 1; k < 4; ++k) L.tw.push_back(compute_twiddle(i * k, cross));
    }
    return L;
}


#ifdef QD_DEV_FAST
#define QD_FMT_CASES(X) case 0: return X(0);
#else
#define QD_FMT_CASES(X) case 0: return X(0); case 1: return X(1); case 2: return X(2); case 3: return X(3);
#endif

constexpr int dyn_lb(int nco) { return nco == 2 ? 3 : 4; }
template <int F, int NCO, bool FI, class G = DynGeo>
chain_fn pick_dyn(bool aligned) {
    return aligned ? k_chain<F, NCO, G, FI, 4, false, true, dyn_lb(NCO)> : k_chain<F, NCO, G, FI, 4, false, false, dyn_lb(NCO)>;
}

template <int F>
chain_fn pick_fmt(int nco, bool fir, bool aligned, bool windowed) {
    if (windowed && fir) {
        switch (nco) {
        case 0: return pick_dyn<F, 0, true, WinGeo>(aligned);
        case 1: return pick_dyn<F, 1, true, WinGeo>(aligned);
        default: return pick_dyn<F, 2, true, WinGeo>(aligned);
        }
    }
    switch (nco) {
    case 0: return fir ? pick_dyn<F, 0, true>(aligned) : pick_dyn<F, 0, false>(aligned);
    case 1: return fir ? pick_dyn<F, 1, true>(aligned) : pick_dyn<F, 1, false>(aligned);
    default: return fir ? pick_dyn<F, 2, true>(aligned) : pick_dyn<F, 2, false>(aligned);
    }
}

chain_fn pick_generic(int fmt, int nco, bool fir, bool aligned, bool windowed = false) {
#define QD_X(F) pick_fmt<F>(nco, fir, aligned, windowed)
    switch (fmt) { QD_FMT_CASES(QD_X) }
#undef QD_X
    return nullptr;
}

template <int F>
chain_fn pick_rows_fmt(int nco, bool fir) {
    switch (nco) {
    case 0: return fir ? k_chain<F, 0, RowGeo, true, 4, false, false, dyn_lb(0)> : k_chain<F, 0, RowGeo, false, 4, false, false, dyn_lb(0)>;
    case 1: return fir ? k_chain<F, 1, RowGeo, true, 4, false, false, dyn_lb(1)> : k_chain<F, 1, RowGeo, false, 4, false, false, dyn_lb(1)>;
    default: return fir ? k_chain<F, 2, RowGeo, true, 4, false, false, dyn_lb(2)> : k_chain<F, 2, RowGeo, false, 4, false, false, dyn_lb(2)>;
    }
}
// ... 83 lines not shown
    return h;
}
bool read_file(const std::string &path, std::vector<char> *out) {
    FILE *f = fopen(path.c_str(), "rb");
    if (!f) return false;
    fseek(f, 0, SEEK_END); long n = ftell(f); fseek(f, 0, SEEK_SET);
    if (n < 0) { fclose(f); return false; }
    out->resize((size_t)n);
    const bool ok = n == 0 || fread(out->data(), 1, (size_t)n, f) == (size_t)n;
    fclose(f);
    return ok;
}
std::string jit_cache_dir() {
    std::string d;
    if (const char *e = getenv("QD_JIT_CACHE")) {
        if (!*e || !strcmp(e, "0") || !strcmp(e, "off")) return "";
        d = e;
    } else if (const char *x = getenv("XDG_CACHE_HOME")) { if (*x) d = std::string(x) + "/quadrs_hip"; }
    if (d.empty()) { const char *h = getenv("HOME"); if (!h || !*h) return ""; d = std::string(h) + "/.cache/quadrs_hip"; }
    for (size_t i = 1; i <= d.size(); ++i)
        if (i == d.size() || d[i] == '/') (void)mkdir(d.substr(0, i).c_str(), 0755);
    return d;
}

hipFunction_t jit_chain_kernel(const JitKey &k, std::string *why, bool may_compile = true) {
    std::lock_guard<std::mutex> lock(g_jit_mu);
    int jit_dev = 0;
    (void)hipGetDevice(&jit_dev);
    const std::pair<int, JitKey> dk(jit_dev, k);
    auto it = g_jit_cache.find(dk);
    if (it != g_jit_cache.end()) return it->second;
    if (auto bad = g_jit_failed.find(dk); bad != g_jit_failed.end()) { *why = bad->second; return nullptr; }
    const std::string dir = csrc_dir();
    std::vector<char> hdrs[3];
    const char *const hdr_names[3] = {"/qd_chain.h", "/qd_device.h", "/qd_geometry.h"};
    for (int i = 0; i < 3; ++i)
        if (!read_file(dir + hdr_names[i], &hdrs[i])) {
            *why = "kernel headers not found next to the library (" + dir + ")";
            return nullptr;
        }
    char geo[160], tail[64], name[512];
    snprintf(geo, sizeof geo, "qd::FixedGeo<%u, %u, %u, %u, %u, %u, %u, %u, %u, %u>", k.W, k.S, k.D, k.T, k.G, k.firb, k.firr, k.pad, k.batch, k.flags);
    const Family fam = family_of(k.flags);
    switch (fam) {
    case kFamSpark0: case kFamSpark2: snprintf(tail, sizeof tail, "%d, %d", k.lb, k.epi); break;
    case kFamSpark: snprintf(tail, sizeof tail, "%d, %d, %d", k.rch, k.lb, k.epi); break;
    case kFamPipe3s: snprintf(tail, sizeof tail, "%d, %d, %d", k.rch, k.lb, k.nt); break;
    case kFamPipe3: snprintf(tail, sizeof tail, "%d, %d", k.rch, k.lb); break;
    default: snprintf(tail, sizeof tail, "%s, %d, %s, true, %d, %d", k.fir ? "true" : "false", k.rch, k.whole ? "true" : "false", k.lb, k.nt); break;
    }
    if (fam == kFamSpark0) snprintf(name, sizeof name, "%s<%d, %s, %s>", family_name(k.flags), k.fmt, geo, tail);
    else snprintf(name, sizeof name, "%s<%d, %d, %s, %s>", family_name(k.flags), k.fmt, k.nco, geo, tail);
    const std::string src = std::string("#include \"qd_chain.h\"\ntemplate __global__ void ") + name + "(const qd::ChainParams);\n";
    hiprtcProgram prog;
    if (hiprtcCreateProgram(&prog, src.c_str(), "qd_jit.hip", 0, nullptr, nullptr) != HIPRTC_SUCCESS) { *why = "hiprtcCreateProgram failed"; return nullptr; }
    hiprtcAddNameExpression(prog, name);
    const std::string inc = "-I" + dir;
    const char *opts[] = {"--offload-arch=gfx950", "-O3", "-ffp-contract=off", "-fno-fast-math", "-std=c++17", inc.c_str(),
                          "-mllvm", "-amdgpu-atomic-optimizer-strategy=None"};
    std::vector<const char *> optv(opts, opts + sizeof opts / sizeof opts[0]);
#ifdef QD_STAMP
    optv.push_back("-DQD_STAMP");
#endif
#ifdef QD_DEVELOP
    optv.push_back("-DQD_DEVELOP");
#endif
#ifdef QD_WGTIME
    optv.push_back("-DQD_WGTIME");
#endif
// ... 115 lines not shown
    unsigned long long *work = nullptr;
    void *cmp_tmp = nullptr;
    size_t cmp_tmp_bytes = 0;
    hipEvent_t done = nullptr;
    bool launched = false;
};

struct qd_plan {
    qd_chain_desc d{};
    qd_plan_options opt{};
    int device = 0;
    bool has_shift = false, has_fir = false;
    uint32_t W = 0, logW = 0, S = 0, D = 1, T = 0;
    uint32_t blk_len = 0, blk_subs = 1;
    uint32_t tile_extra = 0;
    uint64_t dec_len = 0, n_windows = 0, out_rate = 0;
    double ratio = 0.0;
    std::vector<float> taps_h;
    float *taps_d = nullptr;
    FftLayout fft;
    float2 *tw_d = nullptr;
    Geometry geo;
    chain_fn fn = nullptr, fn_unaligned = nullptr;
    const FixedEntry *fixed = nullptr;
    bool spark = false;
    uint32_t spark_ts = 0;
    uint32_t spark_R = 0;
    uint32_t phase_unit = 1;
    hipFunction_t jit_fn = nullptr;
    int wg_per_cu = 1, n_cu = 256, prefetch_mode = 2, nco = 0, nt = kThreads;
    int launch_nt = kThreads;
    uint32_t kflags = 0;
    uint32_t dbg = 0;
    double2 *jtab_d = nullptr, *jtab256_d = nullptr;
    NcoTabs tabs_dev, tabs_slot[2];
    const uint64_t *row_offsets_d = nullptr;
    const float *window_d = nullptr;
    float *win_own_d = nullptr;
    bool rows = false, rows_blue = false;
    RowTab rows_tab512;
    bool timing = false, ev_made = false, ev_recorded = false;
    hipEvent_t ev0{}, ev1{};
    void *pin_in[2] = {nullptr, nullptr}, *pin_out[2] = {nullptr, nullptr};
    void *dev_in[2] = {nullptr, nullptr}, *dev_out[2] = {nullptr, nullptr};
    size_t stage_in_bytes = 0, stage_out_bytes = 0, pin_in_bytes = 0, pin_out_bytes = 0;
    hipStream_t streams[2] = {nullptr, nullptr};
    qd_plan_stats stats{};
    qd_plan *cmp_a = nullptr, *cmp_b = nullptr;
    bool casc = false;
    uint32_t c_D1 = 1, c_T1 = 0, c_D2 = 1, c_T2 = 0, c_n2 = 0, c_M = 0, c_flags = 0, c_inter = 0, c_src = 0;
    double c_ratio[3] = {0, 0, 0};
    uint64_t c_complete = 0;
    size_t c_lds = 0;
    int c_wg_per_cu = 1;
    float *c_h1 = nullptr, *c_h2 = nullptr;
    double2 *c_jtab = nullptr;
    std::vector<qd_stage> stages;
    std::vector<std::vector<float>> stage_taps;
    std::vector<qd_plan *> shards;
    std::vector<qd_shard_info> shard_info;
    std::mutex mu;
};
static Family plan_family(const qd_plan *p) { return (p->jit_fn || p->fixed || p->spark) ? family_of(p->kflags) : kFamChain; }
static bool plan_on_rows(const qd_plan *p) { return (p->jit_fn || p->fixed || p->spark) && row_aligned(p->kflags); }

namespace {

uint64_t out_bytes_per_window(const qd_plan *p) {
    switch (p->d.epilogue) {
    case QD_EPI_NORMS_F32: return (uint64_t)p->W * 4;
    case QD_EPI_GLYPH_U8: return p->W;
    case QD_EPI_CF32_BLOCKS: return (uint64_t)p->blk_len * 8;
    case QD_EPI_ROWS_F32: return (uint64_t)p->blk_len * 4;
    default: return 1;
    }
}

int rows_slice(uint64_t len, uint64_t W, int has_slice, uint64_t *start, uint64_t *end, uint64_t output_len) {
    if (!has_slice) {
        if (len < W) return fail(QD_ERR_PANIC, "len < width underflows (src/ffts.rs:29)");
        *start = 0; *end = len - W;
    }
    if (!(*end > *start)) return fail(QD_ERR_PANIC, "Invalid slice: end (%llu) must be greater than start (%llu)", (unsigned long long)*end, (unsigned long long)*start);
    if (!(*end < len)) return fail(QD_ERR_PANIC, "Slice end (%llu) exceeds sample length (%llu)", (unsigned long long)*end, (unsigned long long)len);
    const uint64_t visible = *end - *start;
    if (!(visible > output_len)) return fail(QD_ERR_INVALID, "Visible samples (%llu) must be greater than output length (%llu)", (unsigned long long)visible, (unsigned long long)output_len);
    return QD_OK;
}
uint64_t rows_offset(uint64_t start, uint64_t end, uint64_t output_len, uint64_t i) {
// ... 468 lines not shown
    if (W >= 512 && (uint64_t)T >= 4ull * D && rules(1, fl_tile, 2, 2, 4, S & ~1u).kPackedTile) {
        const uint32_t fl_half = fl_tile | kGeoHalfTile | kGeoFastP1 | kGeoNtLoads, fl_rows = fl_tile | kGeoFastP1 | kGeoNtLoads | kGeoNtInner;
        const FixedRules h = rules(1, fl_half, 2, 2, 4);
        const bool half_ok = W >= 1024 && h.kHalfTile && on_rows(h, 512);
        const int nt = half_ok ? 512 : (W >= 1024 ? 1024 : 512);
        const uint32_t fl = half_ok ? fl_half : (on_rows(rules(1, fl_rows, 2, 2, 4), nt) ? fl_rows : fl_tile);
        if (lds_for(1, W, S, D, T_lds, nullptr, 2, 2, lut8, fl) > kLdsMax) return false;
        r->G = 1; r->nt = nt; r->batch = 2; r->flags = fl; r->firr = 2; r->firb = 4;
        return true;
    }
    if (W <= 256) {
        const uint32_t g = W >= 128 ? 1u : 128u / W;
        const FixedRules d2 = rules(g, kGeoNoSplit | kGeoDeferFft, 2);
        if (!d2.kPairFir) return false;
        const bool defer = d2.defer_fft_ok(true, 256);
        const uint32_t bt = defer ? 2u : 1u, fl_base = kGeoNoSplit | (defer ? kGeoDeferFft : 0u), fl_rows = fl_base | kGeoFastP1 | kGeoNtLoads | kGeoNtInner;
        const uint32_t fl = on_rows(rules(g, fl_rows, bt), 256) ? fl_rows : fl_base;
        if (p->n_windows < g || lds_for(g, W, S, D, T_lds, nullptr, 2, bt, lut8, fl) > kLdsMax / 2) return false;
        r->G = g; r->nt = 256; r->batch = bt; r->flags = fl;
        return true;
    }
    return false;
}

std::vector<Candidate> chain_candidates_of(const qd_plan *p, uint32_t T_lds, bool windowed) {
    const qd_chain_desc &d = p->d;
    const int policy = p->opt.kernel_policy, spl = spl_of(d.format), bps = bps_of(d.format);
    const uint32_t W = p->W, S = p->S;
    const bool write_sink = d.epilogue == QD_EPI_CF32_BLOCKS;
    const bool jit_ok = policy != QD_KERNEL_GENERIC && policy != QD_KERNEL_NO_PLAN_TIME;
    Candidate plain;
    plain.G = plain_tiles(p, T_lds);
    Candidate generic = plain;
    generic.wg_regs = dyn_lb(p->nco);
    const FixedEntry *fixed = (p->has_fir && !write_sink && policy != QD_KERNEL_GENERIC && !windowed) ? find_fixed(d.format, p->nco, W, S, p->D, p->T) : nullptr;
    const bool fast = d.mode == QD_MODE_FAST && p->has_fir && jit_ok && !write_sink;
    Candidate recipe;
    const bool has_recipe = jit_ok && p->has_fir && (!fixed || fast) && geometry_recipe(p, T_lds, &recipe);
    Candidate table;
    if (fixed) {
        table.src = Candidate::kTable; table.fixed = fixed;
        table.G = fixed->G; table.nt = fixed->nt; table.pad = (uint32_t)fixed->pad; table.batch = (uint32_t)fixed->batch;
        table.flags = (uint32_t)fixed->flags; table.lb = fixed->lb; table.wg_regs = std::max(1, fixed->lb * 256 / fixed->nt);
        if (!has_recipe) return {table};
    }
    if (has_recipe) {
        if (fast) recipe.flags |= kGeoFastFma;
        if (fixed) return {chain_build(p, recipe, true), table};
        if (write_sink) return {chain_build(p, recipe, true), generic};
        return {chain_build(p, recipe, true), chain_build(p, plain, false), generic};
    }
    if (jit_ok && !write_sink && p->has_fir && (uint64_t)p->T >= 8ull * p->D) {
        auto outs = [&](uint32_t g) { return S < W ? (uint64_t)(g - 1) * S + W : (uint64_t)g * W; };
        Candidate lf;
        lf.nt = 512; lf.pad = 2; lf.lb = 2; lf.noslp = 1;
        while (lf.G < 64 && outs(lf.G + 1) <= 512 && lds_for(lf.G + 1, W, S, p->D, T_lds, nullptr, 2, 1, lut8_of(d.format)) <= kLdsMax) ++lf.G;
        if (p->n_windows && lf.G > p->n_windows) lf.G = (uint32_t)p->n_windows;
        return {chain_build(p, lf, true), chain_build(p, plain, false), generic};
    }
    auto spark = [&](uint32_t ts, uint32_t flags, int lb) {
        Candidate c;
        c.src = Candidate::kBuiltinSpark; c.spark_ts = ts; c.G = ts / W; c.nt = (int)(kSparkRow / spl); c.flags = kGeoSpark | flags; c.lb = c.wg_regs = lb;
        return c;
    };
    auto spark_build = [&](Candidate c, int nco, uint32_t key_S, int rch) {
        c.src = Candidate::kBuild;
        c.key = JitKey{d.format, nco, 0, rch, 1, c.lb, kThreads, W, key_S, 1, 0, c.G, 8, 1, 0, 1, 1, c.flags, d.epilogue};
// ... 241 lines not shown
        break;
    }
    if (!won) return fail(QD_ERR_UNSUPPORTED, "no kernel for this chain");

    hipDeviceProp_t prop;
    if (hipGetDeviceProperties(&prop, p->device) == hipSuccess) p->n_cu = prop.multiProcessorCount;
    const int by_lds = (int)(kLdsMax / (p->geo.lds_main ? p->geo.lds_main : p->geo.lds_bytes));
    p->wg_per_cu = std::min(4, std::max(1, by_lds));
    if (won->wg_regs) p->wg_per_cu = std::min(p->wg_per_cu, won->wg_regs);
    if (p->launch_nt > kThreads) p->wg_per_cu = std::min(p->wg_per_cu, 2048 / p->launch_nt);
    if (hinted && h[7] && (int)h[7] < p->wg_per_cu) p->wg_per_cu = (int)h[7];
    if (const char *e = dev_env("QD_WG_PER_CU")) { int v = atoi(e); if (v >= 1 && v <= 8) p->wg_per_cu = v; }
    if (p->jit_fn) {
        if (hipError_t e = hipFuncSetAttribute(reinterpret_cast<const void *>(p->jit_fn), hipFuncAttributeMaxDynamicSharedMemorySize, (int)kLdsMax); e != hipSuccess)
            return fail(QD_ERR_HIP, "hipFuncSetAttribute(plan-time kernel, max dynamic LDS %zu): %s", kLdsMax, hipGetErrorString(e));
    }
    for (chain_fn f : {p->fn, p->fn_unaligned}) {
        hipError_t e = hipFuncSetAttribute(reinterpret_cast<const void *>(f), hipFuncAttributeMaxDynamicSharedMemorySize, (int)kLdsMax);
        if (e != hipSuccess)
            return fail(QD_ERR_HIP, "hipFuncSetAttribute(max dynamic LDS %zu): %s", kLdsMax, hipGetErrorString(e));
    }

    p->fft = fft_layout(d.width);
    if (!p->fft.tw.empty()) {
        HIPCHK(hipMalloc(&p->tw_d, p->fft.tw.size() * sizeof(float2)));
        HIPCHK(hipMemcpy(p->tw_d, p->fft.tw.data(), p->fft.tw.size() * sizeof(float2), hipMemcpyHostToDevice));
    }
    if (p->has_fir) {
        HIPCHK(hipMalloc(&p->taps_d, p->T * sizeof(float)));
        HIPCHK(hipMemcpy(p->taps_d, p->taps_h.data(), p->T * sizeof(float), hipMemcpyHostToDevice));
    }
    if (p->has_shift) {
        const uint32_t ROW = p->nt * spl_of(d.format);
        HIPCHK(hipMalloc(&p->jtab_d, ROW * sizeof(double2)));
        hipLaunchKernelGGL(k_jtab, dim3((ROW + 255) / 256), dim3(256), 0, 0, p->ratio, ROW, p->jtab_d);
        HIPCHK(hipGetLastError());
        if (p->nt != kThreads) {
            const uint32_t ROW256 = kThreads * spl_of(d.format);
            HIPCHK(hipMalloc(&p->jtab256_d, ROW256 * sizeof(double2)));
            hipLaunchKernelGGL(k_jtab, dim3((ROW256 + 255) / 256), dim3(256), 0, 0, p->ratio, ROW256, p->jtab256_d);
            HIPCHK(hipGetLastError());
        }
        HIPCHK(hipDeviceSynchronize());
    }
    return QD_OK;
}


namespace {
struct DeviceGuard {
    int prev = -1; bool switched = false;
    explicit DeviceGuard(int dev) {
        if (hipGetDevice(&prev) == hipSuccess && prev != dev) switched = hipSetDevice(dev) == hipSuccess;
    }
    ~DeviceGuard() { if (switched) (void)hipSetDevice(prev); }
};

void partition_windows(uint64_t n_windows, uint32_t n_shards, uint64_t step, uint64_t rpw, uint32_t tile, std::vector<qd_shard_info> *out) {
    out->assign(n_shards, qd_shard_info{});
    uint64_t per = (n_windows + n_shards - 1) / n_shards;
    per = (per + tile - 1) / tile * tile;
    const uint64_t total_end = n_windows ? (n_windows - 1) * step + rpw : 0;
    for (uint32_t g = 0; g < n_shards; ++g) {
        qd_shard_info &s = (*out)[g];
        s.w0 = std::min<uint64_t>(n_windows, (uint64_t)g * per);
        s.w1 = std::min<uint64_t>(n_windows, (uint64_t)(g + 1) * per);
        uint64_t own_first = s.w0 * step;
        uint64_t own_end = (g + 1 < n_shards && s.w1 < n_windows) ? s.w1 * step : total_end;
        if (s.w1 == s.w0) { own_first = total_end; own_end = total_end; }
        const uint64_t need_end = s.w1 > s.w0 ? (s.w1 - 1) * step + rpw : own_first;
        s.own_first = own_first;
        s.own_count = own_end > own_first ? own_end - own_first : 0;
// ... 139 lines not shown
                }
            }
            return false;
        };
        fits = pick(kLdsMax / 4, 64) || pick(kLdsMax, 1);
        p->blk_len = B; p->blk_subs = B / p->W;
        p->logW = ilog2(p->W); p->S = p->W;
    } else {
        fits = sub_tile(g.n2, g.n2);
    }
    if (!fits) return fail(QD_ERR_UNSUPPORTED, "cascade: %zu bytes of LDS per workgroup exceed the %zu available", p->c_lds, kLdsMax);
    int by_lds = (int)(kLdsMax / p->c_lds);
    p->c_wg_per_cu = by_lds < 1 ? 1 : (by_lds > 8 ? 8 : by_lds);
    hipDeviceProp_t prop;
    if (hipGetDeviceProperties(&prop, p->device) == hipSuccess) p->n_cu = prop.multiProcessorCount;
    for (const void *f : {reinterpret_cast<const void *>(k_cascade<0>), reinterpret_cast<const void *>(k_cascade<1>),
                          reinterpret_cast<const void *>(k_cascade<2>), reinterpret_cast<const void *>(k_cascade<3>),
                          reinterpret_cast<const void *>(k_cascade_write<0>), reinterpret_cast<const void *>(k_cascade_write<1>),
                          reinterpret_cast<const void *>(k_cascade_write<2>), reinterpret_cast<const void *>(k_cascade_write<3>)})
        if (hipError_t e = hipFuncSetAttribute(f, hipFuncAttributeMaxDynamicSharedMemorySize, (int)kLdsMax); e != hipSuccess)
            return fail(QD_ERR_HIP, "hipFuncSetAttribute(k_cascade, max dynamic LDS %zu): %s", kLdsMax, hipGetErrorString(e));
    if (!write) p->fft = fft_layout(d.width);
    if (!p->fft.tw.empty()) {
        HIPCHK(hipMalloc(&p->tw_d, p->fft.tw.size() * sizeof(float2)));
        HIPCHK(hipMemcpy(p->tw_d, p->fft.tw.data(), p->fft.tw.size() * sizeof(float2), hipMemcpyHostToDevice));
    }
    p->taps_h = p->stage_taps[g.l1];
    HIPCHK(hipMalloc(&p->c_h1, g.T1 * sizeof(float)));
    HIPCHK(hipMemcpy(p->c_h1, p->stage_taps[g.l1].data(), g.T1 * sizeof(float), hipMemcpyHostToDevice));
    if (l2) {
        HIPCHK(hipMalloc(&p->c_h2, g.T2 * sizeof(float)));
        HIPCHK(hipMemcpy(p->c_h2, p->stage_taps[g.l2].data(), g.T2 * sizeof(float), hipMemcpyHostToDevice));
    }
    HIPCHK(hipMalloc(&p->c_jtab, 3 * kCascadeRow * sizeof(double2)));
    HIPCHK(hipMemset(p->c_jtab, 0, 3 * kCascadeRow * sizeof(double2)));
    for (int k = 0; k < 3; ++k)
        if (sidx[k] >= 0) {
            hipLaunchKernelGGL(k_jtab, dim3((kCascadeRow + 255) / 256), dim3(256), 0, 0, p->c_ratio[k], kCascadeRow, p->c_jtab + k * kCascadeRow);
            HIPCHK(hipGetLastError());
        }
    HIPCHK(hipDeviceSynchronize());
    return QD_OK;
}

void stage_taps_of(const qd_stage *st, size_t n, const StageGeo &g, std::vector<std::vector<float>> *t) {
    t->assign(n, {});
    for (size_t i = 0; i < n; ++i)
        if (st[i].kind == QD_STAGE_LOWPASS) { (*t)[i].resize(st[i].taps); design_taps(st[i].lowpass_hz, g.in_rate[i], st[i].taps, (*t)[i].data()); }
}
}

int qd_stages_geometry(const qd_chain_desc *desc, const qd_stage *stages, size_t n_stages, qd_plan_info *info, uint64_t *complete) {
    if (!info || !complete) return fail(QD_ERR_INVALID, "info/complete is NULL");
    StageGeo g;
    int rc = stages_geo(desc, stages, n_stages, &g);
    if (rc) return rc;
    const qd_chain_desc &d = *desc;
    const bool write = d.epilogue == QD_EPI_CF32_BLOCKS;
    if (write && g.routed) return fail(QD_ERR_UNSUPPORTED, "qd_stages_geometry: the write sink's blocks are the one-stage plan's (qd_plan_get_info)");
    if (g.routed) {
        g.complete = g.n_windows;
        g.n2 = (uint32_t)d.width;
    }
    memset(info, 0, sizeof *info);
    info->n_windows = g.n_windows;
    info->decimated_len = g.len;
    info->out_sample_rate = g.rate;
    info->out_bytes_per_window = write ? d.width * 8 : (d.epilogue == QD_EPI_NORMS_F32 || d.epilogue == QD_EPI_ROWS_F32) ? d.width * 4 : (d.epilogue == QD_EPI_GLYPH_U8 ? d.width : 1);
// ... 34 lines not shown
    p->rows_blue = !pow2;
    p->blk_len = (uint32_t)d.width;
    p->logW = ilog2(d.width); p->W = 1u << p->logW;
    p->S = p->W + (p->has_fir ? (p->T + p->D - 1) / p->D : 0);
    p->nt = kThreads; p->launch_nt = kThreads;
    hipDeviceProp_t prop;
    if (hipGetDeviceProperties(&prop, p->device) == hipSuccess) p->n_cu = prop.multiProcessorCount;
    const int fmt = d.format;
    if (pow2 || p->has_fir) {
        uint32_t raw_elems = 0;
        p->geo.lds_bytes = rows_tile(p->W, p->S, p->D, p->T, lut8_of(fmt), &p->geo.G, &raw_elems);
        if (p->geo.lds_bytes > kLdsMax || (uint64_t)raw_elems * p->D >= (1ull << 32))
            return fail(QD_ERR_UNSUPPORTED, "one row (W*D+T = %llu samples) exceeds the 160 KiB LDS tile", (unsigned long long)((uint64_t)d.width * p->D + p->T));
        p->geo.lds_main = p->geo.lds_bytes; p->geo.lds_raw_elems = raw_elems;
        p->geo.Dp = p->D + ((p->D % 2 == 0) ? 1 : 0);
        p->wg_per_cu = std::min(4, std::max(1, (int)(kLdsMax / p->geo.lds_bytes)));
        p->fn = p->fn_unaligned = pick_rows(fmt, p->nco, p->has_fir);
        if (!p->fn) return fail(QD_ERR_UNSUPPORTED, "no kernel built for this format (QD_DEV_FAST build?)");
        if (hipError_t e = hipFuncSetAttribute(reinterpret_cast<const void *>(p->fn), hipFuncAttributeMaxDynamicSharedMemorySize, (int)kLdsMax); e != hipSuccess)
            return fail(QD_ERR_HIP, "hipFuncSetAttribute(max dynamic LDS %zu): %s", kLdsMax, hipGetErrorString(e));
        p->fft = fft_layout(p->W);
        if (!p->fft.tw.empty()) {
            HIPCHK(hipMalloc(&p->tw_d, p->fft.tw.size() * sizeof(float2)));
            HIPCHK(hipMemcpy(p->tw_d, p->fft.tw.data(), p->fft.tw.size() * sizeof(float2), hipMemcpyHostToDevice));
        }
    }
    if (p->has_fir) {
        p->taps_h.resize(p->T); design_taps(d.lowpass_hz, d.sample_rate, p->T, p->taps_h.data());
        HIPCHK(hipMalloc(&p->taps_d, p->T * sizeof(float)));
        HIPCHK(hipMemcpy(p->taps_d, p->taps_h.data(), p->T * sizeof(float), hipMemcpyHostToDevice));
    }
    if (p->has_shift) {
        const uint32_t ROW = kThreads * spl_of(fmt);
        HIPCHK(hipMalloc(&p->jtab_d, ROW * sizeof(double2)));
        hipLaunchKernelGGL(k_jtab, dim3((ROW + 255) / 256), dim3(256), 0, 0, p->ratio, ROW, p->jtab_d);
        HIPCHK(hipGetLastError());
        HIPCHK(hipDeviceSynchronize());
    }
    return QD_OK;
}

int window_init(qd_plan *p) {
    std::vector<float> win;
    blackman_harris(p->d.width, &win);
    HIPCHK(hipMalloc(&p->win_own_d, win.size() * sizeof(float)));
    HIPCHK(hipMemcpy(p->win_own_d, win.data(), win.size() * sizeof(float), hipMemcpyHostToDevice));
    p->window_d = p->win_own_d;
    return QD_OK;
}

int composite_init(qd_plan *p, uint64_t rate) {
    if (p->opt.n_shards > 1) return fail(QD_ERR_UNSUPPORTED, "a window larger than the LDS tile runs as a two-stage plan, which is not sharded inside one process");
    const qd_chain_desc &d = p->d;
    qd_plan_options copt = p->opt;
    copt.n_shards = 0;
    memset(copt.tile_hint, 0, sizeof copt.tile_hint);
    qd_chain_desc a = d;
    a.stride = d.width; a.epilogue = QD_EPI_CF32_BLOCKS; a.has_range = 0;
    a.windowing = 0;
    int rc = qd_plan_create_ex(&a, &copt, &p->cmp_a);
    if (rc) return rc;
    qd_chain_desc b{};
    b.struct_size = sizeof b;
    b.format = QD_FMT_CF32; b.sample_rate = rate ? rate : 1;
    b.n_samples = d.epilogue == QD_EPI_BUCKET2_U8 ? (p->n_windows + 1) * d.width : p->n_windows * d.width + 1;
    b.width = d.width; b.stride = d.width; b.epilogue = d.epilogue; b.mode = d.mode;
    b.has_range = d.has_range; b.range_min = d.range_min; b.range_max = d.range_max;
// ... 754 lines not shown
    const void *src = bytes; void *dst = out;
    if (mem != QD_MEM_DEVICE) {
        void *di = nullptr, *dout = nullptr;
        int rc = ws.get(0, ib, &di); if (rc) return rc;
        rc = ws.get(1, ob, &dout); if (rc) return rc;
        HIPCHK(hipMemcpyAsync(di, bytes, ib, hipMemcpyHostToDevice, st));
        src = di; dst = dout;
    }
    size_t blocks = (n_pairs + 255) / 256; if (blocks > 65536) blocks = 65536;
    hipLaunchKernelGGL(k_unpack, dim3((uint32_t)blocks), dim3(256), 0, st, fmt, static_cast<const uint8_t *>(src), n_pairs,
                       static_cast<float2 *>(dst));
    HIPCHK(hipGetLastError());
    if (mem != QD_MEM_DEVICE) HIPCHK(hipMemcpyAsync(out, dst, ob, hipMemcpyDeviceToHost, st));
    return finish_call(mem, st);
}

int qd_shift(qd_c32 *buf, size_t n, uint64_t abs_off, double ratio, int mem) {
    if (n == 0) return QD_OK;
    if (!buf) return fail(QD_ERR_INVALID, "NULL buffer");
    constexpr uint32_t ROW = 512;
    const hipStream_t st = g_stream;
    WsLease ws(st);
    if (ws.rc) return ws.rc;
    float2 *d = reinterpret_cast<float2 *>(buf);
    if (mem != QD_MEM_DEVICE) {
        void *db = nullptr;
        int rc = ws.get(0, n * 8, &db); if (rc) return rc;
        HIPCHK(hipMemcpyAsync(db, buf, n * 8, hipMemcpyHostToDevice, st));
        d = static_cast<float2 *>(db);
    }
    const uint64_t r0 = abs_off / ROW, r1 = (abs_off + n + ROW - 1) / ROW, rows = r1 - r0;
    void *rt = nullptr, *jt = nullptr;
    int rc = ws.get(2, rows * sizeof(RowBase), &rt); if (rc) return rc;
    rc = ws.get(3, ROW * sizeof(double2), &jt); if (rc) return rc;
    hipLaunchKernelGGL(k_rowtab, dim3((uint32_t)((rows + 255) / 256)), dim3(256), 0, st, ratio, ROW, r0, rows, (uint64_t)0, static_cast<RowBase *>(rt));
    hipLaunchKernelGGL(k_jtab, dim3(2), dim3(256), 0, st, ratio, ROW, static_cast<double2 *>(jt));
    const int so = (std::fabs(ratio) * (double)(abs_off + n) > 268435456.0) ? 1 : 0;
    const uint32_t grid = (uint32_t)(rows < 4096 ? rows : 4096);
    hipLaunchKernelGGL(k_shift, dim3(grid), dim3(256), 0, st, d, abs_off, (uint64_t)n, ratio, static_cast<const RowBase *>(rt), r0, rows,
                       static_cast<const double2 *>(jt), so);
    HIPCHK(hipGetLastError());
    if (mem != QD_MEM_DEVICE) HIPCHK(hipMemcpyAsync(buf, d, n * 8, hipMemcpyDeviceToHost, st));
    return finish_call(mem, st);
}

int qd_lowpass_block(const float *taps, size_t T, uint64_t D, const qd_c32 *raw, size_t valid, qd_c32 *out,
                     size_t out_cap, size_t *produced, int mem) {
    if (!taps || !raw || !out || !produced) return fail(QD_ERR_INVALID, "NULL argument");
    if (T < 2 || D == 0) return fail(QD_ERR_PANIC, "size < 2 or decimate 0 (src/filter.rs:47,74)");
    if (valid < T) return fail(QD_ERR_PANIC, "valid < filter.len(): usize underflow at src/filter.rs:76");
    size_t out_n = (size_t)((uint64_t)(valid - T) / D);
    if (out_n > out_cap) return fail(QD_ERR_PANIC, "buf too small for %zu outputs (src/filter.rs:78-80)", out_n);
    *produced = out_n;
    if (out_n == 0) return QD_OK;
    const hipStream_t st = g_stream;
    WsLease ws(st);
    if (ws.rc) return ws.rc;
    void *dt = nullptr;
    int rc = ws.get(2, T * 4, &dt); if (rc) return rc;
    HIPCHK(hipMemcpyAsync(dt, taps, T * 4, hipMemcpyHostToDevice, st));
    HIPCHK(hipStreamSynchronize(st));
    const float2 *r = reinterpret_cast<const float2 *>(raw);
    float2 *o = reinterpret_cast<float2 *>(out);
    if (mem != QD_MEM_DEVICE) {
        void *dr = nullptr, *dout = nullptr;
        rc = ws.get(0, valid * 8, &dr); if (rc) return rc;
        rc = ws.get(1, out_n * 8, &dout); if (rc) return rc;
        HIPCHK(hipMemcpyAsync(dr, raw, valid * 8, hipMemcpyHostToDevice, st));
        r = static_cast<const float2 *>(dr); o = static_cast<float2 *>(dout);
    }
    size_t blocks = (out_n + 127) / 128; if (blocks > 65536) blocks = 65536;
    hipLaunchKernelGGL(k_lowpass_block, dim3((uint32_t)blocks), dim3(128), 0, st, static_cast<const float *>(dt), (uint32_t)T, D, r,
                       (uint64_t)valid, o, (uint64_t)out_n);
// ... 1670 lines not shown
            t = taps_of.insert({{c.lowpass_hz, c.taps}, (uint64_t)taps_h.size()}).first;
            taps_h.resize(taps_h.size() + c.taps);
            design_taps(c.lowpass_hz, sample_rate, c.taps, taps_h.data() + t->second);
        }
        j.taps_at = t->second;
        if (c.shift_hz != 0) {
            j.ratio = qd_shift_ratio(c.shift_hz, sample_rate);
            auto l = lane_of.find(c.shift_hz);
            if (l == lane_of.end()) { l = lane_of.insert({c.shift_hz, (uint64_t)lane_ratio.size()}).first; lane_ratio.push_back(j.ratio); }
            j.lane_at = l->second * kCutsNcoRow;
            j.flags = kCutShift | ((std::fabs(j.ratio) * (double)(j.span0 + j.valid) > 268435456.0) ? kCutSecondOrder : 0u);
        }
    }
    std::vector<CutBatch> batches;
    cuts_batches(cuts, n_cuts, std::max<uint64_t>(1, (opt.chunk_bytes ? opt.chunk_bytes : kCutsDefaultChunk) / bps), &batches);

    int dev = 0;
    (void)hipGetDevice(&dev);
    const void *anchor = src_mem == QD_MEM_DEVICE ? src : (out_mem == QD_MEM_DEVICE ? (const void *)out : nullptr);
    if (anchor) {
        hipPointerAttribute_t at;
        if (hipPointerGetAttributes(&at, anchor) == hipSuccess) dev = at.device;
        else (void)hipGetLastError();
    }
    DeviceGuard guard(dev);
    const hipStream_t st = static_cast<hipStream_t>(stream);
    WsLease ws(st);
    if (ws.rc) return ws.rc;
    const bool src_dev = src_mem == QD_MEM_DEVICE, out_dev = out_mem == QD_MEM_DEVICE;
    const size_t n_lane = lane_ratio.size();
    const size_t jobs_b = (jobs.size() * sizeof(CutJob) + 15) & ~(size_t)15, taps_b = (taps_h.size() * 4 + 15) & ~(size_t)15, ratio_b = (n_lane * 8 + 15) & ~(size_t)15;
    void *tab_d = nullptr, *lane_d = nullptr;
    int rc = ws.get(2, jobs_b + taps_b + ratio_b, &tab_d); if (rc) return rc;
    rc = ws.get(3, std::max<size_t>(n_lane, 1) * kCutsNcoRow * sizeof(double2), &lane_d); if (rc) return rc;
    char *const tab = static_cast<char *>(tab_d);
    HIPCHK(hipMemcpyAsync(tab, jobs.data(), jobs.size() * sizeof(CutJob), hipMemcpyHostToDevice, st));
    HIPCHK(hipMemcpyAsync(tab + jobs_b, taps_h.data(), taps_h.size() * 4, hipMemcpyHostToDevice, st));
    if (n_lane) HIPCHK(hipMemcpyAsync(tab + jobs_b + taps_b, lane_ratio.data(), n_lane * 8, hipMemcpyHostToDevice, st));
    const CutJob *jobs_d = reinterpret_cast<const CutJob *>(tab);
    const float *taps_d = reinterpret_cast<const float *>(tab + jobs_b);
    const double *ratio_d = reinterpret_cast<const double *>(tab + jobs_b + taps_b);

    const void *fn = fmt == 0 ? reinterpret_cast<const void *>(k_cuts<0>) : fmt == 1 ? reinterpret_cast<const void *>(k_cuts<1>)
                   : fmt == 2 ? reinterpret_cast<const void *>(k_cuts<2>) : reinterpret_cast<const void *>(k_cuts<3>);
    HIPCHK(hipFuncSetAttribute(fn, hipFuncAttributeMaxDynamicSharedMemorySize, (int)kCutsLdsBytes));

    std::vector<std::vector<CutTile>> kept;
    kept.reserve(batches.size());
    std::vector<qd_c32> down;
    bool first_batch = true;
    for (const CutBatch &b : batches) {
        kept.emplace_back();
        std::vector<CutTile> &tiles = kept.back();
        cuts_tiles(cuts, b, out_dev, offs.data(), src_dev, src_first, &tiles);
        const uint32_t n_tiles = (uint32_t)tiles.size();
        const size_t tiles_b = ((size_t)n_tiles * sizeof(CutTile) + 31) & ~(size_t)31;
        void *batch_d = nullptr, *in_d = nullptr, *out_d = nullptr;
        rc = ws.get(4, tiles_b + (size_t)n_tiles * kCutsTileRows * sizeof(RowBase), &batch_d); if (rc) return rc;
        HIPCHK(hipMemcpyAsync(batch_d, tiles.data(), (size_t)n_tiles * sizeof(CutTile), hipMemcpyHostToDevice, st));
        const CutTile *tiles_d = static_cast<const CutTile *>(batch_d);
        RowBase *rows_d = reinterpret_cast<RowBase *>(static_cast<char *>(batch_d) + tiles_b);
        const uint8_t *in = static_cast<const uint8_t *>(src);
        if (!src_dev) {
            rc = ws.get(0, b.src_samples * bps + 16, &in_d); if (rc) return rc;
            for (const CutSpan &sp : b.spans)
                HIPCHK(hipMemcpyAsync(static_cast<char *>(in_d) + sp.at * bps, static_cast<const char *>(src) + (sp.first - src_first) * bps, sp.count * bps,
                                      hipMemcpyHostToDevice, st));
            in = static_cast<const uint8_t *>(in_d);
        }
        float2 *o = reinterpret_cast<float2 *>(out);
        if (!out_dev) {
            rc = ws.get(1, b.out_samples * 8, &out_d); if (rc) return rc;
            o = static_cast<float2 *>(out_d);
        }
        const uint32_t lanes = first_batch ? (uint32_t)n_lane : 0u;
        const uint64_t table_threads = (uint64_t)n_tiles * kCutsTileRows + (uint64_t)lanes * kCutsNcoRow;
        hipLaunchKernelGGL(k_cuts_tables, dim3((uint32_t)((table_threads + 255) / 256)), dim3(256), 0, st, jobs_d, tiles_d, n_tiles, rows_d, ratio_d, lanes,
                           static_cast<double2 *>(lane_d));
        const RowBase *rows_c = rows_d;
        const double2 *lane_c = static_cast<const double2 *>(lane_d);
        switch (fmt) {
        case 0: hipLaunchKernelGGL(k_cuts<0>, dim3(n_tiles), dim3(kCutsThreads), kCutsLdsBytes, st, in, jobs_d, tiles_d, taps_d, rows_c, lane_c, o); break;
        case 1: hipLaunchKernelGGL(k_cuts<1>, dim3(n_tiles), dim3(kCutsThreads), kCutsLdsBytes, st, in, jobs_d, tiles_d, taps_d, rows_c, lane_c, o); break;
        case 2: hipLaunchKernelGGL(k_cuts<2>, dim3(n_tiles), dim3(kCutsThreads), kCutsLdsBytes, st, in, jobs_d, tiles_d, taps_d, rows_c, lane_c, o); break;
        default: hipLaunchKernelGGL(k_cuts<3>, dim3(n_tiles), dim3(kCutsThreads), kCutsLdsBytes, st, in, jobs_d, tiles_d, taps_d, rows_c, lane_c, o); break;
        }
        HIPCHK(hipGetLastError());
        first_batch = false;
        if (!out_dev) {
            down.resize(b.out_samples);
            HIPCHK(hipMemcpyAsync(down.data(), out_d, b.out_samples * 8, hipMemcpyDeviceToHost, st));
            HIPCHK(hipStreamSynchronize(st));
            for (const CutPiece &p : b.pieces) memcpy(out + offs[p.cut] + p.first, down.data() + p.out_at, (size_t)p.count * 8);
        }
    }
    HIPCHK(hipStreamSynchronize(st));
    return QD_OK;
}

int qd_cuts_run(int fmt, uint64_t sample_rate, uint64_t n_samples, const void *src, int src_mem, uint64_t src_first, uint64_t src_count,
                const qd_cut *cuts, size_t n_cuts, qd_c32 *out, int out_mem, const qd_plan_options *options, void *stream) {
    return cuts_run_impl(fmt, sample_rate, n_samples, src, src_mem, src_first, src_count, cuts, n_cuts, out, out_mem, options, stream, false);
}


int qd_symbols_geometry(const qd_symbols_desc *desc, const qd_segment *segments, size_t n, uint64_t *offsets) {
    std::string err;
    if (const int rc = symbols_check(desc, segments, n, false, 0, offsets, nullptr, nullptr, &err)) return fail(rc, "%s", err.c_str());
    return QD_OK;
}

static int symbols_device_of(const void *a, bool a_dev, const void *b, bool b_dev) {
    int dev = 0;
// ... 186 lines not shown
```

Before: 650,700.

## Precompute c+s sums in NCO row and lane tables to cut FMAs

Moves the NCO table code into a new header. The row table's pad slot now stores a precomputed c+s term, and lane entries grow to 24 bytes with an extra field, so the complex rotation can use fewer multiplies (a Gauss-style three-multiply form). The LDS lane-table sizing changes to match. It also lowers launch bounds for the dyn chain with NCO=1 and format 3. The cost is more table bandwidth and LDS per entry, plus possible small changes in rounding.

Result: faster. 659,900 (median of 6 runs) (+1.4%).

```diff
diff --git a/quadrs_amd/build.py b/quadrs_amd/build.py
--- a/quadrs_amd/build.py
+++ b/quadrs_amd/build.py
@@ -5,7 +5,7 @@
 HERE = os.path.dirname(os.path.abspath(__file__))
 ROOT = os.path.dirname(HERE)
 SRC = [(os.path.join(HERE, "csrc", "quadrs_hip.hip"), [])]
-DEPS = [s for s, _ in SRC] + [os.path.join(HERE, "csrc", f) for f in ("qd_chain.h", "qd_cascade.h", "qd_device.h", "qd_geometry.h", "qd_registry.h", "qd_summary.h", "qd_pieces.h", "qd_pool.h", "qd_limbs.h", "qd_mean.h", "qd_power.h", "qd_spread.h", "qd_density.h", "qd_bands.h", "qd_paint.h", "qd_lists.h", "qd_bursts.h", "qd_emissions.h", "qd_cuts.h", "qd_cuts_plan.h", "qd_symbols.h", "qd_symbols_plan.h")] + [
+DEPS = [s for s, _ in SRC] + [os.path.join(HERE, "csrc", f) for f in ("qd_chain.h", "qd_cascade.h", "qd_device.h", "qd_nco.h", "qd_geometry.h", "qd_registry.h", "qd_summary.h", "qd_pieces.h", "qd_pool.h", "qd_limbs.h", "qd_mean.h", "qd_power.h", "qd_spread.h", "qd_density.h", "qd_bands.h", "qd_paint.h", "qd_lists.h", "qd_bursts.h", "qd_emissions.h", "qd_cuts.h", "qd_cuts_plan.h", "qd_symbols.h", "qd_symbols_plan.h")] + [
     os.path.join(ROOT, "include", "quadrs_hip.h")]
 OBJ_DIR = os.path.join(ROOT, "build", "obj")
 OUT = os.path.join(HERE, "libquadrs_hip.so")
diff --git a/quadrs_amd/csrc/qd_cascade.h b/quadrs_amd/csrc/qd_cascade.h
--- a/quadrs_amd/csrc/qd_cascade.h
+++ b/quadrs_amd/csrc/qd_cascade.h
@@ -11,7 +11,7 @@
 struct CascadeParams {
     ChainParams c;
     const float *h1, *h2;
-    const double2 *jtab;
+    const LaneEntry *jtab;
     const RowBase *rows[3];
     uint64_t row0[3];
     double ratio0, ratio1, ratio2;
@@ -87,12 +87,9 @@
     else { const uint32_t w = reinterpret_cast<const uint32_t *>(src)[i]; return make_float2(unpack_cs16(w & 0xffffu), unpack_cs16(w >> 16)); }
 }
 
-__device__ __forceinline__ float2 casc_nco(const RowBase *rb, uint64_t row0, uint64_t n, const double2 *jt, double ratio) {
+__device__ __forceinline__ float2 casc_nco(const RowBase *rb, uint64_t row0, uint64_t n, const LaneEntry *jt, double ratio) {
     const uint32_t j = (uint32_t)(n % kCascadeRow);
-    const double2 cs = jt[j];
-    LaneRot lr;
-    lr.jf = (double)j; lr.c = cs.x; lr.s = cs.y;
-    return nco_mul<true>(rb[n / kCascadeRow - row0], lr, ratio);
+    return nco_mul<true>(rb[n / kCascadeRow - row0], nco_lane_rot((double)j, jt[j]), ratio);
 }
 
 template <int FMT>
diff --git a/quadrs_amd/csrc/qd_chain.h b/quadrs_amd/csrc/qd_chain.h
--- a/quadrs_amd/csrc/qd_chain.h
+++ b/quadrs_amd/csrc/qd_chain.h
@@ -46,7 +46,7 @@
     void *out;
     const RowBase *rowtab;
     uint64_t rowtab_row0;
-    const double2 *jtab;
+    const LaneEntry *jtab;
     const float *taps;
     const float2 *tw;
     double ratio;
@@ -283,16 +283,23 @@
     return v;
 }
 
+template <bool LOAD_CS>
 __device__ __forceinline__ RowBase load_rowbase(const ChainParams &P, uint64_t r) {
     const_f64_p rp = (const_f64_p)(uintptr_t)(P.rowtab + (r - P.rowtab_row0));
     RowBase rb;
-    rb.c = rp[0]; rb.s = rp[1]; rb.nf = rp[2]; rb.pad_ = 0.0;
+    rb.c = rp[0]; rb.s = rp[1]; rb.nf = rp[2]; rb.cs = 0.0;
+    if constexpr (LOAD_CS) rb.cs = rp[3];
+    return rb;
+}
+template <bool LOAD_CS>
+__device__ __forceinline__ RowBase with_cs(RowBase rb) {
+    if constexpr (!LOAD_CS) rb.cs = rb.c + rb.s;
     return rb;
 }
 
 __device__ __forceinline__ RowBase load_rowbase_at(const_f64_p tile_rows, uint32_t i) {
     RowBase rb;
-    rb.c = tile_rows[4 * i + 0]; rb.s = tile_rows[4 * i + 1]; rb.nf = tile_rows[4 * i + 2]; rb.pad_ = 0.0;
+    rb.c = tile_rows[4 * i + 0]; rb.s = tile_rows[4 * i + 1]; rb.nf = tile_rows[4 * i + 2]; rb.cs = tile_rows[4 * i + 3];
     return rb;
 }
 
@@ -1089,10 +1096,7 @@
 #pragma unroll
         for (int u = 0; u < SPL; ++u) {
             uint32_t j = first + u;
-            double2 cs = P.jtab[j];
-            lr[u].jf = (double)j;
-            lr[u].c = cs.x;
-            lr[u].s = cs.y;
+            lr[u] = nco_lane_rot((double)j, P.jtab[j]);
         }
     };
     if constexpr (HAS_SHIFT && !kReloadLane) load_lane_rot(tid * SPL);
@@ -1254,8 +1258,8 @@
                 for (uint32_t r = 0; r < wg.n_rows; ++r) {
                     const Vec v = fetch_row<FMT, NT, false>(P, wg, r, tid);
                     RowBase rb{};
-                    if constexpr (HAS_SHIFT) rb = load_rowbase(P, wg.r0 + r);
-                    process_row_any<FMT, NT, NCO>(P, geo, wg, r, tid, v, rb, lr, lane_pad, lut, rawg);
+                    if constexpr (HAS_SHIFT) rb = load_rowbase<GeoT::kFixed>(P, wg.r0 + r);
+                    process_row_any<FMT, NT, NCO>(P, geo, wg, r, tid, v, with_cs<GeoT::kFixed>(rb), lr, lane_pad, lut, rawg);
                 }
             }
         } else
@@ -1314,7 +1318,7 @@
             if (!ng.valid) ng = tg;
             rt_pf = prefetch_rowtab<HAS_SHIFT>(P, ng, tid);
             RowBase rb_next{};
-            if constexpr (HAS_SHIFT) rb_next = load_rowbase(P, tg.r0);
+            if constexpr (HAS_SHIFT) rb_next = load_rowbase<GeoT::kFixed>(P, tg.r0);
 #pragma unroll
             for (int i = 0; i < RCH; ++i) {
                 const Vec v = pf[i];
@@ -1329,9 +1333,9 @@
                     QD_STAMP_ROW(2);
 #endif
                     if constexpr (HAS_SHIFT) {
-                        if ((uint32_t)i + 1 < tg.n_rows) rb_next = load_rowbase(P, tg.r0 + i + 1);
+                        if ((uint32_t)i + 1 < tg.n_rows) rb_next = load_rowbase<GeoT::kFixed>(P, tg.r0 + i + 1);
                     }
-                    process_row_any<FMT, NT, NCO>(P, geo, tg, i, tid, v, rb, lr, lane_pad, lut, raw);
+                    process_row_any<FMT, NT, NCO>(P, geo, tg, i, tid, v, with_cs<GeoT::kFixed>(rb), lr, lane_pad, lut, raw);
                     QD_STAMP_ROW(3);
                 }
                 __builtin_amdgcn_sched_barrier(0);
@@ -1357,11 +1361,11 @@
 #pragma unroll
                 for (int i = 0; i < RCH; ++i) {
                     rb[i] = RowBase{};
-                    if constexpr (HAS_SHIFT) { if (r + i < tg.n_rows) rb[i] = load_rowbase(P, tg.r0 + r + i); }
+                    if constexpr (HAS_SHIFT) { if (r + i < tg.n_rows) rb[i] = load_rowbase<GeoT::kFixed>(P, tg.r0 + r + i); }
                 }
 #pragma unroll
                 for (int i = 0; i < RCH; ++i)
-                    if (r + i < tg.n_rows) process_row_any<FMT, NT, NCO>(P, geo, tg, r + i, tid, cur[i], rb[i], lr, lane_pad, lut, raw);
+                    if (r + i < tg.n_rows) process_row_any<FMT, NT, NCO>(P, geo, tg, r + i, tid, cur[i], with_cs<GeoT::kFixed>(rb[i]), lr, lane_pad, lut, raw);
             }
         }
         QD_STAMP_AT(0);
@@ -1890,8 +1894,7 @@
 #pragma unroll
             for (int u = 0; u < SPL; ++u) {
                 const uint32_t j = tid * SPL + u;
-                const double2 cs = P.jtab[j];
-                lr[u].jf = (double)j; lr[u].c = cs.x; lr[u].s = cs.y;
+                lr[u] = nco_lane_rot((double)j, P.jtab[j]);
             }
         }
         const uint32_t lane_pad = pad_index(geo, tid * SPL);
@@ -2211,8 +2214,7 @@
 #pragma unroll
             for (int u = 0; u < SPL; ++u) {
                 const uint32_t j = tid * SPL + u;
-                const double2 cs = P.jtab[j];
-                lr[u].jf = (double)j; lr[u].c = cs.x; lr[u].s = cs.y;
+                lr[u] = nco_lane_rot((double)j, P.jtab[j]);
             }
         }
         const uint32_t lane_pad = pad_index(geo, tid * SPL);
@@ -2456,6 +2458,8 @@
 
 template <class GeoT, bool F = GeoT::kFixed> struct W_CT_GE8 { static constexpr bool value = false; };
 template <class GeoT> struct W_CT_GE8<GeoT, true> { static constexpr bool value = GeoT::W >= 8; };
+static_assert(sizeof(LaneEntry) == kLaneEntryBytes, "the lane table's entry as qd_geometry.h sizes it");
+constexpr uint32_t kSparkLaneLds = kSparkRow * kLaneEntryBytes / 8;
 template <int FMT> struct SparkTraits {
     using FT = FmtTraits<FMT>;
     static constexpr uint32_t SPL = FT::SPL, CH = 64u * SPL, RQ = kSparkRow / CH;
@@ -2480,8 +2484,8 @@
     const uint32_t tid = threadIdx.x, lane = tid & 63u;
     const uint32_t wave = __builtin_amdgcn_readfirstlane(tid >> 6);
     constexpr bool kLdsLane = HAS_SHIFT && GeoT::kFixed;
-    double2 *jt = reinterpret_cast<double2 *>(twl + (W < 32u ? 32u : W));
-    float2 *fbw = twl + (W < 32u ? 32u : W) + (kLdsLane ? 2u * kSparkRow : 0u) + (size_t)wave * TS;
+    LaneEntry *jt = reinterpret_cast<LaneEntry *>(twl + (W < 32u ? 32u : W));
+    float2 *fbw = twl + (W < 32u ? 32u : W) + (kLdsLane ? kSparkLaneLds : 0u) + (size_t)wave * TS;
     {
         const uint32_t n_tw = W - geo.base_len;
         for (uint32_t i = tid; i < n_tw; i += kThreads) twl[i] = P.tw[i];
@@ -2511,7 +2515,7 @@
             for (int i = 0; i < NCH * SPL; ++i) pos[i] ^= SZ::delta(pos[i]);
         }
     }
-    double2 lcs[HAS_SHIFT && !kLdsLane ? RQ * SPL : 1];
+    LaneEntry lcs[HAS_SHIFT && !kLdsLane ? RQ * SPL : 1];
     double ljf[HAS_SHIFT ? SPL : 1];
     if constexpr (HAS_SHIFT) {
         if constexpr (!kLdsLane) {
@@ -2604,8 +2608,7 @@
                 LaneRot lr[SPL];
 #pragma unroll
                 for (int u = 0; u < SPL; ++u) {
-                    const double2 cs = kLdsLane ? jt[(uint32_t)q * CH + lane * SPL + (uint32_t)u] : lcs[kLdsLane ? 0 : q * SPL + u];
-                    lr[u].jf = ljf[u]; lr[u].c = cs.x; lr[u].s = cs.y;
+                    lr[u] = nco_lane_rot(ljf[u], kLdsLane ? jt[(uint32_t)q * CH + lane * SPL + (uint32_t)u] : lcs[kLdsLane ? 0 : q * SPL + u]);
                 }
                 RowBase rbq = rb;
                 rbq.nf = rb.nf + (double)(q * (int)CH);
@@ -2730,10 +2733,10 @@
 
     extern __shared__ __attribute__((aligned(16))) char smem[];
     float2 *twl = reinterpret_cast<float2 *>(smem);
-    double2 *jt = reinterpret_cast<double2 *>(twl + W);
+    LaneEntry *jt = reinterpret_cast<LaneEntry *>(twl + W);
     const uint32_t tid = threadIdx.x, lane = tid & 63u;
     const uint32_t wave = __builtin_amdgcn_readfirstlane(tid >> 6);
-    float2 *fbw = twl + W + (HAS_SHIFT ? 2u * kSparkRow : 0u) + (size_t)wave * TS;
+    float2 *fbw = twl + W + (HAS_SHIFT ? kSparkLaneLds : 0u) + (size_t)wave * TS;
     for (uint32_t i = tid; i < W - base; i += kThreads) twl[i] = P.tw[i];
     if constexpr (HAS_SHIFT) { for (uint32_t i = tid; i < kSparkRow; i += kThreads) jt[i] = P.jtab[i]; }
     __syncthreads();
@@ -2818,8 +2821,7 @@
                 if constexpr (HAS_SHIFT) {
                     const uint32_t jrow = (W >= kSparkRow ? 0u : (g * W) % kSparkRow) + (y * width) % kSparkRow;
                     const uint32_t j = jrow + 2 * xp + (uint32_t)u;
-                    const double2 cs = jt[j];
-                    LaneRot lr; lr.jf = (double)j; lr.c = cs.x; lr.s = cs.y;
+                    const LaneRot lr = nco_lane_rot((double)j, jt[j]);
                     const RowBase &rb = rbl[W > kSparkRow ? (y * width) / kSparkRow : 0];
                     x = cmul_pk(x, nco_mul<NCO == 2>(rb, lr, P.ratio));
                 }
diff --git a/quadrs_amd/csrc/qd_cuts.h b/quadrs_amd/csrc/qd_cuts.h
--- a/quadrs_amd/csrc/qd_cuts.h
+++ b/quadrs_amd/csrc/qd_cuts.h
@@ -24,7 +24,7 @@
 }
 
 __global__ __launch_bounds__(256) void k_cuts_tables(const CutJob *__restrict__ jobs, const CutTile *__restrict__ tiles, uint32_t n_tiles, RowBase *__restrict__ rowtab,
-                                                    const double *__restrict__ lane_ratio, uint32_t n_lane, double2 *__restrict__ lanetab) {
+                                                    const double *__restrict__ lane_ratio, uint32_t n_lane, LaneEntry *__restrict__ lanetab) {
     const uint64_t i = (uint64_t)blockIdx.x * blockDim.x + threadIdx.x;
     const uint64_t n_row = (uint64_t)n_tiles * kCutsTileRows;
     if (i < n_row) {
@@ -36,16 +36,10 @@
         cut_tile_reads(jb, tl, &lo, &hi);
         const uint64_t row = (jb.span0 + lo) / kCutsNcoRow + r;
         if (row * kCutsNcoRow >= jb.span0 + hi) return;
-        RowBase rb;
-        rb.nf = (double)(row * kCutsNcoRow);
-        rb.pad_ = 0.0;
-        nco_table_entry(rb.nf, jb.ratio, &rb.c, &rb.s);
-        rowtab[i] = rb;
+        rowtab[i] = nco_row_entry((double)(row * kCutsNcoRow), jb.ratio);
     } else if (i - n_row < (uint64_t)n_lane * kCutsNcoRow) {
         const uint64_t u = (i - n_row) / kCutsNcoRow, j = (i - n_row) % kCutsNcoRow;
-        double c, s;
-        nco_table_entry((double)j, lane_ratio[u], &c, &s);
-        lanetab[u * kCutsNcoRow + j] = make_double2(c, s);
+        lanetab[u * kCutsNcoRow + j] = nco_lane_entry((double)j, lane_ratio[u]);
     }
 }
 
@@ -86,7 +80,7 @@
 template <int FMT>
 __global__ __launch_bounds__(kCutsThreads) void k_cuts(const uint8_t *__restrict__ src, const CutJob *__restrict__ jobs, const CutTile *__restrict__ tiles,
                                                        const float *__restrict__ taps, const RowBase *__restrict__ rowtab,
-                                                       const double2 *__restrict__ lanetab, float2 *__restrict__ out) {
+                                                       const LaneEntry *__restrict__ lanetab, float2 *__restrict__ out) {
     extern __shared__ __attribute__((aligned(32))) char smem_cuts[];
     RowBase *rows = reinterpret_cast<RowBase *>(smem_cuts);
     float2 *xs = reinterpret_cast<float2 *>(smem_cuts + kCutsTileRows * sizeof(RowBase));
@@ -108,9 +102,7 @@
             const uint64_t n = abs0 + k;
             const uint32_t j = (uint32_t)(n % kCutsNcoRow);
             const RowBase rb = rows[(uint32_t)(n / kCutsNcoRow - row0)];
-            const double2 cs = lanetab[jb.lane_at + j];
-            LaneRot lr;
-            lr.jf = (double)j; lr.c = cs.x; lr.s = cs.y;
+            const LaneRot lr = nco_lane_rot((double)j, lanetab[jb.lane_at + j]);
             const float2 m = second ? nco_mul<true>(rb, lr, jb.ratio) : nco_mul<false>(rb, lr, jb.ratio);
             v = cmul(v, m);
         }
diff --git a/quadrs_amd/csrc/qd_device.h b/quadrs_amd/csrc/qd_device.h
--- a/quadrs_amd/csrc/qd_device.h
+++ b/quadrs_amd/csrc/qd_device.h
@@ -160,67 +160,15 @@
     return r;
 }
 
-
-struct __attribute__((aligned(32))) RowBase {
-    double c, s;
-    double nf;
-    double pad_;
-};
-
-struct LaneRot { double jf, c, s; };
-
-__device__ __forceinline__ void nco_table_entry(double kf, double ratio, double *c, double *s) {
-    const double th = kf * ratio;
-    const double lo = __builtin_fma(kf, ratio, -th);
-    double s0, c0;
-    sincos(th, &s0, &c0);
-    const double q = 0.5 * lo * lo, sl = __builtin_fma(-lo * lo * lo, 1.0 / 6.0, lo);
-    *c = c0 + __builtin_fma(-q, c0, -sl * s0);
-    *s = s0 + __builtin_fma(-q, s0, sl * c0);
 }
+#include "qd_nco.h"
+namespace qd {
 
 template <bool SECOND_ORDER>
 __device__ __forceinline__ float2 nco_mul(const RowBase &rb, const LaneRot &lr, double ratio) {
-    const double nf = rb.nf + lr.jf;
-    const double place = nf * ratio;
-    const double r = __builtin_fma(nf, ratio, -place);
-    const double C = __builtin_fma(-rb.s, lr.s, rb.c * lr.c);
-    const double S = __builtin_fma(rb.s, lr.c, rb.c * lr.s);
-    double c, s;
-    if constexpr (SECOND_ORDER) {
-        const double h = 0.5 * r;
-        c = __builtin_fma(r, __builtin_fma(-h, C, S), C);
-        s = __builtin_fma(-r, __builtin_fma(h, S, C), S);
-    } else {
-        c = __builtin_fma(r, S, C);
-        s = __builtin_fma(-r, C, S);
-    }
-    return make_float2((float)c, (float)s);
-}
-
-template <bool SECOND_ORDER, int N>
-__device__ __forceinline__ void nco_mul_n(const RowBase &rb, const LaneRot *lr, double ratio, float2 *m) {
-    double nf[N], pl[N], r[N], C[N], S[N], c[N], s[N];
-#pragma unroll
-    for (int u = 0; u < N; ++u) nf[u] = rb.nf + lr[u].jf;
-#pragma unroll
-    for (int u = 0; u < N; ++u) { pl[u] = nf[u] * ratio; C[u] = rb.c * lr[u].c; S[u] = rb.c * lr[u].s; }
-#pragma unroll
-    for (int u = 0; u < N; ++u) { r[u] = __builtin_fma(nf[u], ratio, -pl[u]); C[u] = __builtin_fma(-rb.s, lr[u].s, C[u]); S[u] = __builtin_fma(rb.s, lr[u].c, S[u]); }
-    if constexpr (SECOND_ORDER) {
-        double h[N], uu[N], vv[N];
-#pragma unroll
-        for (int u = 0; u < N; ++u) h[u] = 0.5 * r[u];
-#pragma unroll
-        for (int u = 0; u < N; ++u) { uu[u] = __builtin_fma(-h[u], C[u], S[u]); vv[u] = __builtin_fma(h[u], S[u], C[u]); }
-#pragma unroll
-        for (int u = 0; u < N; ++u) { c[u] = __builtin_fma(r[u], uu[u], C[u]); s[u] = __builtin_fma(-r[u], vv[u], S[u]); }
-    } else {
-#pragma unroll
-        for (int u = 0; u < N; ++u) { c[u] = __builtin_fma(r[u], S[u], C[u]); s[u] = __builtin_fma(-r[u], C[u], S[u]); }
-    }
-#pragma unroll
-    for (int u = 0; u < N; ++u) m[u] = make_float2((float)c[u], (float)s[u]);
+    float2 m;
+    nco_mul<SECOND_ORDER>(rb, lr, ratio, &m.x, &m.y);
+    return m;
 }
 
 }
diff --git a/quadrs_amd/csrc/qd_geometry.h b/quadrs_amd/csrc/qd_geometry.h
--- a/quadrs_amd/csrc/qd_geometry.h
+++ b/quadrs_amd/csrc/qd_geometry.h
@@ -35,6 +35,7 @@
 constexpr int kPipe3Threads = 1024, kPipe3Prod = 512;
 constexpr uint32_t kSparkRow = 512;
 constexpr uint32_t kSparkMaxW = 1024;
+constexpr uint32_t kLaneEntryBytes = 24;
 
 enum Family { kFamChain, kFamPipe3, kFamPipe3s, kFamSpark, kFamSpark2, kFamSpark0 };
 
@@ -212,7 +213,7 @@
 constexpr uint64_t pipe3_lds_bytes(const FixedRules &g) {
     return 2 * g.lds_raw_alloc * 8 + 4 * g.pipe3_q_pad() * 8 + g.G * g.W * 8 + g.W * 8 + ct_taps_bytes(g.T) + kPipe3QueueBytes;
 }
-constexpr uint64_t spark_lds_bytes(uint64_t W, uint64_t ts, bool lane_table) { return (ct_max(W, 32) + 4 * ts) * 8 + (lane_table ? kSparkRow * 16 : 0); }
+constexpr uint64_t spark_lds_bytes(uint64_t W, uint64_t ts, bool lane_table) { return (ct_max(W, 32) + 4 * ts) * 8 + (lane_table ? kSparkRow * kLaneEntryBytes : 0); }
 constexpr uint64_t kPipe3LdsSlack = 64 - kPipe3QueueBytes, kStreamLdsSlack = 320, kStreamWriteLdsSlack = 64;
 static_assert(31 * 8 < kStreamLdsSlack, "the streaming layout's slack covers FBX_OFF's rounding");
 
diff --git a/quadrs_amd/csrc/qd_nco.h b/quadrs_amd/csrc/qd_nco.h
--- /dev/null
+++ b/quadrs_amd/csrc/qd_nco.h
@@ -0,0 +1,113 @@
+#pragma once
+
+#if defined(__HIPCC_RTC__) || defined(__HIPCC__)
+#define QD_NCO_FN __device__ __forceinline__
+#else
+#include <math.h>
+#define QD_NCO_FN inline
+#endif
+
+namespace qd {
+
+struct __attribute__((aligned(32))) RowBase {
+    double c, s;
+    double nf;
+    double cs;
+};
+
+struct LaneEntry {
+    double c;
+    double sum;
+    double dif;
+};
+
+struct LaneRot { double jf, c, sum, dif; };
+
+QD_NCO_FN void nco_table_entry(double kf, double ratio, double *c, double *s) {
+    const double th = kf * ratio;
+    const double lo = __builtin_fma(kf, ratio, -th);
+    double s0, c0;
+    sincos(th, &s0, &c0);
+    const double q = 0.5 * lo * lo, sl = __builtin_fma(-lo * lo * lo, 1.0 / 6.0, lo);
+    *c = c0 + __builtin_fma(-q, c0, -sl * s0);
+    *s = s0 + __builtin_fma(-q, s0, sl * c0);
+}
+
+QD_NCO_FN RowBase nco_row_entry(double nf, double ratio) {
+    RowBase rb;
+    rb.nf = nf;
+    nco_table_entry(nf, ratio, &rb.c, &rb.s);
+    rb.cs = rb.c + rb.s;
+    return rb;
+}
+
+QD_NCO_FN LaneEntry nco_lane_entry(double jf, double ratio) {
+    double c, s;
+    nco_table_entry(jf, ratio, &c, &s);
+    LaneEntry e;
+    e.c = c; e.sum = c + s; e.dif = s - c;
+    return e;
+}
+
+QD_NCO_FN LaneRot nco_lane_rot(double jf, const LaneEntry &e) {
+    LaneRot lr;
+    lr.jf = jf; lr.c = e.c; lr.sum = e.sum; lr.dif = e.dif;
+    return lr;
+}
+
+QD_NCO_FN void nco_rotate(const RowBase &rb, const LaneRot &lr, double *C, double *S) {
+    const double k = lr.c * rb.cs;
+    *C = __builtin_fma(-rb.s, lr.sum, k);
+    *S = __builtin_fma(rb.c, lr.dif, k);
+}
+
+template <bool SECOND_ORDER>
+QD_NCO_FN void nco_mul_f64(const RowBase &rb, const LaneRot &lr, double ratio, double *c, double *s) {
+    const double nf = rb.nf + lr.jf;
+    const double place = nf * ratio;
+    const double r = __builtin_fma(nf, ratio, -place);
+    double C, S;
+    nco_rotate(rb, lr, &C, &S);
+    if constexpr (SECOND_ORDER) {
+        const double h = 0.5 * r;
+        *c = __builtin_fma(r, __builtin_fma(-h, C, S), C);
+        *s = __builtin_fma(-r, __builtin_fma(h, S, C), S);
+    } else {
+        *c = __builtin_fma(r, S, C);
+        *s = __builtin_fma(-r, C, S);
+    }
+}
+
+template <bool SECOND_ORDER>
+QD_NCO_FN void nco_mul(const RowBase &rb, const LaneRot &lr, double ratio, float *re, float *im) {
+    double c, s;
+    nco_mul_f64<SECOND_ORDER>(rb, lr, ratio, &c, &s);
+    *re = (float)c; *im = (float)s;
+}
+
+template <bool SECOND_ORDER, int N, class F2>
+QD_NCO_FN void nco_mul_n(const RowBase &rb, const LaneRot *lr, double ratio, F2 *m) {
+    double nf[N], pl[N], r[N], k[N], C[N], S[N], c[N], s[N];
+#pragma unroll
+    for (int u = 0; u < N; ++u) nf[u] = rb.nf + lr[u].jf;
+#pragma unroll
+    for (int u = 0; u < N; ++u) { pl[u] = nf[u] * ratio; k[u] = lr[u].c * rb.cs; }
+#pragma unroll
+    for (int u = 0; u < N; ++u) { r[u] = __builtin_fma(nf[u], ratio, -pl[u]); C[u] = __builtin_fma(-rb.s, lr[u].sum, k[u]); S[u] = __builtin_fma(rb.c, lr[u].dif, k[u]); }
+    if constexpr (SECOND_ORDER) {
+        double h[N], uu[N], vv[N];
+#pragma unroll
+        for (int u = 0; u < N; ++u) h[u] = 0.5 * r[u];
+#pragma unroll
+        for (int u = 0; u < N; ++u) { uu[u] = __builtin_fma(-h[u], C[u], S[u]); vv[u] = __builtin_fma(h[u], S[u], C[u]); }
+#pragma unroll
+        for (int u = 0; u < N; ++u) { c[u] = __builtin_fma(r[u], uu[u], C[u]); s[u] = __builtin_fma(-r[u], vv[u], S[u]); }
+    } else {
+#pragma unroll
+        for (int u = 0; u < N; ++u) { c[u] = __builtin_fma(r[u], S[u], C[u]); s[u] = __builtin_fma(-r[u], C[u], S[u]); }
+    }
+#pragma unroll
+    for (int u = 0; u < N; ++u) { m[u].x = (float)c[u]; m[u].y = (float)s[u]; }
+}
+
+}
diff --git a/quadrs_amd/csrc/quadrs_hip.hip b/quadrs_amd/csrc/quadrs_hip.hip
--- a/quadrs_amd/csrc/quadrs_hip.hip
+++ b/quadrs_amd/csrc/quadrs_hip.hip
@@ -80,19 +80,13 @@
 __global__ void k_rowtab(double ratio, uint32_t row_len, uint64_t row0, uint64_t n_rows, uint64_t n_off, RowBase *out) {
     uint64_t i = (uint64_t)blockIdx.x * blockDim.x + threadIdx.x;
     if (i >= n_rows) return;
-    RowBase rb;
-    rb.nf = (double)((row0 + i) * (uint64_t)row_len + n_off);
-    rb.pad_ = 0.0;
-    nco_table_entry(rb.nf, ratio, &rb.c, &rb.s);
-    out[i] = rb;
-}
-
-__global__ void k_jtab(double ratio, uint32_t n, double2 *out) {
+    out[i] = nco_row_entry((double)((row0 + i) * (uint64_t)row_len + n_off), ratio);
+}
+
+__global__ void k_jtab(double ratio, uint32_t n, LaneEntry *out) {
     uint32_t j = blockIdx.x * blockDim.x + threadIdx.x;
     if (j >= n) return;
-    double s, c;
-    nco_table_entry((double)j, ratio, &c, &s);
-    out[j] = make_double2(c, s);
+    out[j] = nco_lane_entry((double)j, ratio);
 }
 
 __global__ void k_unpack(int fmt, const uint8_t *src, size_t n, float2 *out) {
@@ -110,14 +104,13 @@
 
 __global__ __launch_bounds__(256) void k_shift(float2 *buf, uint64_t abs_off, uint64_t n, double ratio,
                                                 const RowBase *rowtab, uint64_t row0, uint64_t n_rows,
-                                                const double2 *jtab, int second_order) {
+                                                const LaneEntry *jtab, int second_order) {
     constexpr uint32_t ROW = 512;
     const uint32_t tid = threadIdx.x;
     LaneRot lr[2];
     for (int u = 0; u < 2; ++u) {
         uint32_t j = tid * 2 + u;
-        double2 cs = jtab[j];
-        lr[u].jf = (double)j; lr[u].c = cs.x; lr[u].s = cs.y;
+        lr[u] = nco_lane_rot((double)j, jtab[j]);
     }
     for (uint64_t r = blockIdx.x; r < n_rows; r += gridDim.x) {
         const RowBase rb = rowtab[r];
@@ -169,7 +162,7 @@
 }
 struct BlueSrc {
     const uint8_t *in; uint64_t in_first;
-    double ratio; const RowBase *rowtab; uint64_t rowtab_row0; const double2 *jtab;
+    double ratio; const RowBase *rowtab; uint64_t rowtab_row0; const LaneEntry *jtab;
 };
 template <int FMT, int NCO>
 __global__ __launch_bounds__(256) void k_bluestein(const BlueSrc src, const uint64_t *__restrict__ offs,
@@ -194,8 +187,7 @@
             if constexpr (NCO != 0) {
                 const uint32_t j = (uint32_t)(na & 511u);
                 const RowBase rb = src.rowtab[(na >> 9) - src.rowtab_row0];
-                const double2 cs = src.jtab[j];
-                LaneRot lr; lr.jf = (double)j; lr.c = cs.x; lr.s = cs.y;
+                const LaneRot lr = nco_lane_rot((double)j, src.jtab[j]);
                 xv = cmul_pk(xv, nco_mul<NCO == 2>(rb, lr, src.ratio));
             }
             if (win) xv = cscale(xv, win[n]);
@@ -287,10 +279,10 @@
 #define QD_FMT_CASES(X) case 0: return X(0); case 1: return X(1); case 2: return X(2); case 3: return X(3);
 #endif
 
-constexpr int dyn_lb(int nco) { return nco == 2 ? 3 : 4; }
+constexpr int dyn_lb(int nco, int fmt = 0) { return (nco == 2 || (nco == 1 && fmt == 3)) ? 3 : 4; }
 template <int F, int NCO, bool FI, class G = DynGeo>
 chain_fn pick_dyn(bool aligned) {
-    return aligned ? k_chain<F, NCO, G, FI, 4, false, true, dyn_lb(NCO)> : k_chain<F, NCO, G, FI, 4, false, false, dyn_lb(NCO)>;
+    return aligned ? k_chain<F, NCO, G, FI, 4, false, true, dyn_lb(NCO, F)> : k_chain<F, NCO, G, FI, 4, false, false, dyn_lb(NCO, F)>;
 }
 
 template <int F>
@@ -440,9 +432,9 @@
     if (it != g_jit_cache.end()) return it->second;
     if (auto bad = g_jit_failed.find(dk); bad != g_jit_failed.end()) { *why = bad->second; return nullptr; }
     const std::string dir = csrc_dir();
-    std::vector<char> hdrs[3];
-    const char *const hdr_names[3] = {"/qd_chain.h", "/qd_device.h", "/qd_geometry.h"};
-    for (int i = 0; i < 3; ++i)
+    std::vector<char> hdrs[4];
+    const char *const hdr_names[4] = {"/qd_chain.h", "/qd_device.h", "/qd_geometry.h", "/qd_nco.h"};
+    for (int i = 0; i < 4; ++i)
         if (!read_file(dir + hdr_names[i], &hdrs[i])) {
             *why = "kernel headers not found next to the library (" + dir + ")";
             return nullptr;
@@ -624,7 +616,7 @@
     int launch_nt = kThreads;
     uint32_t kflags = 0;
     uint32_t dbg = 0;
-    double2 *jtab_d = nullptr, *jtab256_d = nullptr;
+    LaneEntry *jtab_d = nullptr, *jtab256_d = nullptr;
     NcoTabs tabs_dev, tabs_slot[2];
     const uint64_t *row_offsets_d = nullptr;
     const float *window_d = nullptr;
@@ -646,7 +638,7 @@
     size_t c_lds = 0;
     int c_wg_per_cu = 1;
     float *c_h1 = nullptr, *c_h2 = nullptr;
-    double2 *c_jtab = nullptr;
+    LaneEntry *c_jtab = nullptr;
     std::vector<qd_stage> stages;
     std::vector<std::vector<float>> stage_taps;
     std::vector<qd_plan *> shards;
@@ -1181,7 +1173,7 @@
     Candidate plain;
     plain.G = plain_tiles(p, T_lds);
     Candidate generic = plain;
-    generic.wg_regs = dyn_lb(p->nco);
+    generic.wg_regs = dyn_lb(p->nco, d.format);
     const FixedEntry *fixed = (p->has_fir && !write_sink && policy != QD_KERNEL_GENERIC && !windowed) ? find_fixed(d.format, p->nco, W, S, p->D, p->T) : nullptr;
     const bool fast = d.mode == QD_MODE_FAST && p->has_fir && jit_ok && !write_sink;
     Candidate recipe;
@@ -1489,12 +1481,12 @@
     }
     if (p->has_shift) {
         const uint32_t ROW = p->nt * spl_of(d.format);
-        HIPCHK(hipMalloc(&p->jtab_d, ROW * sizeof(double2)));
+        HIPCHK(hipMalloc(&p->jtab_d, ROW * sizeof(LaneEntry)));
         hipLaunchKernelGGL(k_jtab, dim3((ROW + 255) / 256), dim3(256), 0, 0, p->ratio, ROW, p->jtab_d);
         HIPCHK(hipGetLastError());
         if (p->nt != kThreads) {
             const uint32_t ROW256 = kThreads * spl_of(d.format);
-            HIPCHK(hipMalloc(&p->jtab256_d, ROW256 * sizeof(double2)));
+            HIPCHK(hipMalloc(&p->jtab256_d, ROW256 * sizeof(LaneEntry)));
             hipLaunchKernelGGL(k_jtab, dim3((ROW256 + 255) / 256), dim3(256), 0, 0, p->ratio, ROW256, p->jtab256_d);
             HIPCHK(hipGetLastError());
         }
@@ -1700,8 +1692,8 @@
         HIPCHK(hipMalloc(&p->c_h2, g.T2 * sizeof(float)));
         HIPCHK(hipMemcpy(p->c_h2, p->stage_taps[g.l2].data(), g.T2 * sizeof(float), hipMemcpyHostToDevice));
     }
-    HIPCHK(hipMalloc(&p->c_jtab, 3 * kCascadeRow * sizeof(double2)));
-    HIPCHK(hipMemset(p->c_jtab, 0, 3 * kCascadeRow * sizeof(double2)));
+    HIPCHK(hipMalloc(&p->c_jtab, 3 * kCascadeRow * sizeof(LaneEntry)));
+    HIPCHK(hipMemset(p->c_jtab, 0, 3 * kCascadeRow * sizeof(LaneEntry)));
     for (int k = 0; k < 3; ++k)
         if (sidx[k] >= 0) {
             hipLaunchKernelGGL(k_jtab, dim3((kCascadeRow + 255) / 256), dim3(256), 0, 0, p->c_ratio[k], kCascadeRow, p->c_jtab + k * kCascadeRow);
@@ -1802,7 +1794,7 @@
     }
     if (p->has_shift) {
         const uint32_t ROW = kThreads * spl_of(fmt);
-        HIPCHK(hipMalloc(&p->jtab_d, ROW * sizeof(double2)));
+        HIPCHK(hipMalloc(&p->jtab_d, ROW * sizeof(LaneEntry)));
         hipLaunchKernelGGL(k_jtab, dim3((ROW + 255) / 256), dim3(256), 0, 0, p->ratio, ROW, p->jtab_d);
         HIPCHK(hipGetLastError());
         HIPCHK(hipDeviceSynchronize());
@@ -2623,13 +2615,13 @@
     const uint64_t r0 = abs_off / ROW, r1 = (abs_off + n + ROW - 1) / ROW, rows = r1 - r0;
     void *rt = nullptr, *jt = nullptr;
     int rc = ws.get(2, rows * sizeof(RowBase), &rt); if (rc) return rc;
-    rc = ws.get(3, ROW * sizeof(double2), &jt); if (rc) return rc;
+    rc = ws.get(3, ROW * sizeof(LaneEntry), &jt); if (rc) return rc;
     hipLaunchKernelGGL(k_rowtab, dim3((uint32_t)((rows + 255) / 256)), dim3(256), 0, st, ratio, ROW, r0, rows, (uint64_t)0, static_cast<RowBase *>(rt));
-    hipLaunchKernelGGL(k_jtab, dim3(2), dim3(256), 0, st, ratio, ROW, static_cast<double2 *>(jt));
+    hipLaunchKernelGGL(k_jtab, dim3(2), dim3(256), 0, st, ratio, ROW, static_cast<LaneEntry *>(jt));
     const int so = (std::fabs(ratio) * (double)(abs_off + n) > 268435456.0) ? 1 : 0;
     const uint32_t grid = (uint32_t)(rows < 4096 ? rows : 4096);
     hipLaunchKernelGGL(k_shift, dim3(grid), dim3(256), 0, st, d, abs_off, (uint64_t)n, ratio, static_cast<const RowBase *>(rt), r0, rows,
-                       static_cast<const double2 *>(jt), so);
+                       static_cast<const LaneEntry *>(jt), so);
     HIPCHK(hipGetLastError());
     if (mem != QD_MEM_DEVICE) HIPCHK(hipMemcpyAsync(buf, d, n * 8, hipMemcpyDeviceToHost, st));
     return finish_call(mem, st);
@@ -4366,7 +4358,7 @@
     const size_t jobs_b = (jobs.size() * sizeof(CutJob) + 15) & ~(size_t)15, taps_b = (taps_h.size() * 4 + 15) & ~(size_t)15, ratio_b = (n_lane * 8 + 15) & ~(size_t)15;
     void *tab_d = nullptr, *lane_d = nullptr;
     int rc = ws.get(2, jobs_b + taps_b + ratio_b, &tab_d); if (rc) return rc;
-    rc = ws.get(3, std::max<size_t>(n_lane, 1) * kCutsNcoRow * sizeof(double2), &lane_d); if (rc) return rc;
+    rc = ws.get(3, std::max<size_t>(n_lane, 1) * kCutsNcoRow * sizeof(LaneEntry), &lane_d); if (rc) return rc;
     char *const tab = static_cast<char *>(tab_d);
     HIPCHK(hipMemcpyAsync(tab, jobs.data(), jobs.size() * sizeof(CutJob), hipMemcpyHostToDevice, st));
     HIPCHK(hipMemcpyAsync(tab + jobs_b, taps_h.data(), taps_h.size() * 4, hipMemcpyHostToDevice, st));
@@ -4410,9 +4402,9 @@
         const uint32_t lanes = first_batch ? (uint32_t)n_lane : 0u;
         const uint64_t table_threads = (uint64_t)n_tiles * kCutsTileRows + (uint64_t)lanes * kCutsNcoRow;
         hipLaunchKernelGGL(k_cuts_tables, dim3((uint32_t)((table_threads + 255) / 256)), dim3(256), 0, st, jobs_d, tiles_d, n_tiles, rows_d, ratio_d, lanes,
-                           static_cast<double2 *>(lane_d));
+                           static_cast<LaneEntry *>(lane_d));
         const RowBase *rows_c = rows_d;
-        const double2 *lane_c = static_cast<const double2 *>(lane_d);
+        const LaneEntry *lane_c = static_cast<const LaneEntry *>(lane_d);
         switch (fmt) {
         case 0: hipLaunchKernelGGL(k_cuts<0>, dim3(n_tiles), dim3(kCutsThreads), kCutsLdsBytes, st, in, jobs_d, tiles_d, taps_d, rows_c, lane_c, o); break;
         case 1: hipLaunchKernelGGL(k_cuts<1>, dim3(n_tiles), dim3(kCutsThreads), kCutsLdsBytes, st, in, jobs_d, tiles_d, taps_d, rows_c, lane_c, o); break;
```
